# Levicoz/Options-model

Measured on AMD Instinct MI355X. Metric: paths x steps / sec (whole American pricing: path-gen + LSM + mean), higher is better.
Workload: dtype f32

## Files before the change

### include/omc.h

```cpp
#ifndef OMC_H
#define OMC_H

#include <stddef.h>
#include <stdint.h>

#ifdef __cplusplus
extern "C" {
#endif

#define OMC_ABI_VERSION 10

typedef struct omc_ctx omc_ctx;

enum {
    OMC_SEM_REFERENCE = 0,
    OMC_SEM_TEXTBOOK = 1,
    OMC_SEM_TWO_PASS = 2
};
enum { OMC_MODEL_GBM = 0, OMC_MODEL_HESTON = 1 };
enum {
    OMC_HESTON_REFERENCE_CLAMP = 0,
    OMC_HESTON_FULL_TRUNCATION = 1,
    OMC_HESTON_CALIBRATOR = 2
};

typedef struct {
    int32_t model;
    int32_t is_put;
    int32_t semantics;
    int32_t antithetic;
    int32_t heston_scheme;
    int32_t n_steps;
    int64_t n_paths;
    double S0, K, r, sigma, T;
    double v0, kappa, theta, xi, rho;
    uint64_t seed;
    uint64_t stream;
    uint64_t pair_offset;
} omc_params;

typedef struct {
    double price;
    double sum, sumsq;
    double std;
    double zero_prob;
    int64_t n_paths, n_exercised, n_zero, sum_nitm;
    double ms_paths, ms_lsm, ms_total;
    double ms_pass1, ms_pass2;
    int64_t timed;
    int64_t folded;
} omc_result;

int omc_abi_version(void);
const char* omc_last_error(void);
int omc_device_count(int* count);
int omc_ctx_device_info(omc_ctx* ctx, int* device, char* pci_bus_id, int pci_len, char* name, int name_len);
int omc_ctx_create(int device, void* hip_stream, omc_ctx** out);
int omc_ctx_destroy(omc_ctx* ctx);
int omc_sync(omc_ctx* ctx);
int omc_alloc(omc_ctx* ctx, size_t bytes, void** dptr);
int omc_free(omc_ctx* ctx, void* dptr);
int omc_memcpy_h2d(omc_ctx* ctx, void* dst, const void* src, size_t bytes);
int omc_memcpy_d2h(omc_ctx* ctx, void* dst, const void* src, size_t bytes);
int omc_set_option(omc_ctx* ctx, const char* key, int64_t value);
int omc_p2p_export(omc_ctx* ctx, void* handle_out, size_t bytes );
int omc_p2p_connect(omc_ctx* ctx, int rank, int world, const void* handles, size_t bytes );
int omc_p2p_disconnect(omc_ctx* ctx);
int omc_p2p_status(omc_ctx* ctx, int* connected, int* world, uint64_t* error_word);

int omc_gbm_paths_f32(omc_ctx* ctx, float* S, int64_t ld, int64_t n_paths, int n_steps, double S0,
                      double r, double sigma, double T, uint64_t seed, uint64_t stream,
                      uint64_t pair_offset, int antithetic);
int omc_heston_paths_f32(omc_ctx* ctx, float* S, int64_t ld, int64_t n_paths, int n_steps,
                         double S0, double r, double T, double v0, double kappa, double theta,
                         double xi, double rho, uint64_t seed, uint64_t stream,
                         uint64_t pair_offset, int scheme);
int omc_gbm_paths_from_normals_f32(omc_ctx* ctx, float* S, int64_t ld, int64_t n_paths,
                                   int n_steps, double S0, double r, double sigma, double T,
                                   const float* Zhalf, int64_t ldz, int antithetic);
int omc_heston_paths_from_normals_f32(omc_ctx* ctx, float* S, int64_t ld, int64_t n_paths,
                                      int n_steps, double S0, double r, double T, double v0,
                                      double kappa, double theta, double xi, double rho,
                                      const float* Z1half, const float* Z2half, int64_t ldz,
                                      int scheme);
int omc_philox4x32_10(omc_ctx* ctx, const uint32_t* in, uint32_t* out, int n);
int omc_gbm_normals_f32(omc_ctx* ctx, float* Z, int64_t ldz, int64_t n_pairs, int n_steps,
                        uint64_t seed, uint64_t stream, uint64_t pair_offset);

int omc_lsm_poly(omc_ctx* ctx, const float* S, int64_t ld, int64_t n_paths, int n_steps, double K,
                 double r, double T, int is_put, int semantics, omc_result* res,
                 double* betas_out, float* sx_out, int32_t* tex_out);
int omc_lsm_apply_frozen(omc_ctx* ctx, const float* S, int64_t ld, int64_t n_paths, int n_steps,
                         double K, double r, double T, int is_put, const double* betas,
                         omc_result* res, float* sx_out, int32_t* tex_out);

int omc_lsm_apply_values(omc_ctx* ctx, const float* S, int64_t ld, int64_t n_paths, int n_steps,
                         double K, double r, double T, int is_put, int semantics, const float* cont,
                         int64_t ldc, omc_result* res, float* sx_out, int32_t* tex_out);

int omc_lsm_contnet(omc_ctx* ctx, const float* S, int64_t ld, int64_t n_paths, int n_steps, double K, double r,
                    double T, int is_put, int nn_hidden, int nn_epochs, double nn_lr, uint64_t nn_seed,
                    omc_result* res, float* sx_out, int32_t* tex_out);
int omc_price_american_contnet(omc_ctx* ctx, const omc_params* p, int nn_hidden, int nn_epochs, double nn_lr,
                               uint64_t nn_seed, omc_result* res);
int omc_contnet_init_params(omc_ctx* ctx, int nn_hidden, int t, uint64_t nn_seed, float* params_out, int n);

typedef int (*omc_allreduce_fn)(void* user, double* dptr, int count);
int omc_set_allreduce_hook(omc_ctx* ctx, omc_allreduce_fn fn, void* user);

int omc_comm_unique_id(void* uid_out, size_t bytes);
int omc_comm_init(omc_ctx* ctx, int rank, int world, const void* uid, size_t bytes);
int omc_comm_destroy(omc_ctx* ctx);
int omc_comm_info(omc_ctx* ctx, int* rank, int* world);
int omc_comm_allreduce_f64(omc_ctx* ctx, double* host_inout, int count, int op);

int omc_price_american(omc_ctx* ctx, const omc_params* p, omc_result* res, float* S_keep,
                       int64_t ld);
typedef struct {
    omc_result base;
    double delta, gamma, vega, rho, theta;
    double se_delta, se_gamma, se_vega, se_rho, se_theta;
    double bump, price_up, price_down;
    int64_t n_exercised_up, n_exercised_down;
    double ms_greeks;
} omc_greeks;
int omc_price_american_greeks(omc_ctx* ctx, const omc_params* p, double bump, const double* betas, double* betas_out,
                              omc_greeks* out);
int omc_price_european(omc_ctx* ctx, const omc_params* p, omc_result* res);

int omc_heston_price_strikes(omc_ctx* ctx, int64_t n_paths, int n_steps, double S0, double r,
                             double T, double v0, double kappa, double theta, double xi, double rho,
                             uint64_t seed, uint64_t stream, int scheme, const double* strikes,
                             int n_strikes, int is_put, double* prices, double* stderrs);
int omc_heston_price_surface(omc_ctx* ctx, int64_t n_paths, int n_steps, double S0, double r, double v0, double kappa,
                             double theta, double xi, double rho, uint64_t seed, int scheme, const double* expiries,
                             const uint64_t* streams, int n_expiries, const double* strikes, const int32_t* expiry_of,
                             int n_quotes, int is_put, double* prices, double* stderrs);

int omc_mlp_param_count(int hidden, int layers);
int omc_lsm_apply_mlp(omc_ctx* ctx, const float* S, int64_t ld, int64_t n_paths, int n_steps, double K,
                      double r, double T, int is_put, int hidden, int layers, const float* params,
                      const double* feat_mean, const double* feat_std, double y_mean, double y_std,
                      double dropout, uint64_t seed, omc_result* res, float* sx_out, int32_t* tex_out);
int omc_lsm_apply_mlp_shard(omc_ctx* ctx, const float* S, int64_t ld, int64_t n_paths, int n_steps, double K,
                      double r, double T, int is_put, int hidden, int layers, const float* params,
                      const double* feat_mean, const double* feat_std, double y_mean, double y_std,
                      double dropout, uint64_t seed, omc_result* res, float* sx_out, int32_t* tex_out,
                            int64_t col_base0, int64_t col_base1);
int omc_nn_build_rows(omc_ctx* ctx, const float* S, int64_t ld, int64_t n_paths, int n_steps, double K,
                      double r, double T, int is_put, float* data, int64_t cap_rows, int64_t* n_rows,
                      double* stats16);
int omc_lsm_ols7(omc_ctx* ctx, const float* S, int64_t ld, int64_t n_paths, int n_steps, double K, double r, double T,
                 int is_put, omc_result* res, double* weights7, double* stats16, float* sx_out, int32_t* tex_out);
int omc_price_american_ols7(omc_ctx* ctx, const omc_params* p, omc_result* res, double* weights7, double* stats16);
int omc_nn_feature_stats(omc_ctx* ctx, const double* x, const int32_t* t, const double* y,
                         int64_t n_rows, double T, double dt, double* out16);
int omc_mlp_train_supported(int hidden, int layers, int64_t batch);
int omc_mlp_train_epoch(omc_ctx* ctx, const float* data, int64_t n_rows, int64_t batch, int hidden,
                        int layers, float* params, float* adam_m, float* adam_v, int64_t* step,
                        double lr, double beta1, double beta2, double eps, double weight_decay,
                        double dropout, uint64_t seed, uint64_t shuffle_key, double* mean_loss);
int omc_mlp_shuffle_indices(omc_ctx* ctx, int64_t n_rows, uint64_t shuffle_key, int64_t* out_device);
int omc_mlp_train_variant(int hidden, int layers, int64_t batch);
int omc_mlp_dropout_masks(omc_ctx* ctx, int variant, int hidden, int layers, int64_t n_rows, const uint32_t* keys,
                          uint32_t step, uint64_t seed, double dropout, uint8_t* out);

int omc_nn_half_counts(omc_ctx* ctx, const float* S, int64_t ld, int64_t n_paths, int n_steps, double K, int is_put,
                       int64_t* counts );
int omc_mlp_shard_epoch(omc_ctx* ctx, const float* data, int64_t n_rows_local, int64_t rows_global, int64_t batch,
                        uint64_t shuffle_key, const int64_t* gstart, const int64_t* lstart, int nseg,
                        int segs_per_step ,
                        float* data_epoch, uint32_t* drop_pos, int64_t* step_off);
int omc_mlp_train_epoch_sharded(omc_ctx* ctx, const float* data_epoch, int64_t n_rows_local, int64_t rows_global,
                                int64_t batch, int hidden, int layers, float* params, float* adam_m, float* adam_v,
                                int64_t* step, double lr, double beta1, double beta2, double eps, double weight_decay,
                                double dropout, uint64_t seed, const int64_t* step_off, const uint32_t* drop_pos,
                                double* mean_loss);

int omc_localvol_param_count(int hidden, int layers);
int omc_localvol_paths_f32(omc_ctx* ctx, float* S, int64_t ld, int64_t n_paths, int n_steps, double S0,
                           double r, double T, double K, int hidden, int layers, const float* params,
                           double m_scale, double tau_scale, double epsilon, const float* Z);

typedef struct {
    const float* data;
    int64_t n_rows, batch;
    float* params;
    float* adam_m;
    float* adam_v;
    int64_t step;
    double lr;
    uint64_t seed;
    uint64_t shuffle_key;
    double mean_loss;
} omc_mlp_job;
int omc_mlp_train_batch_supported(int hidden, int layers, int64_t batch);
int omc_mlp_train_epoch_batch(omc_ctx* ctx, omc_mlp_job* jobs, int n, int hidden, int layers, double beta1,
                              double beta2, double eps, double weight_decay, double dropout);

int omc_price_american_seq(omc_ctx* ctx, const omc_params* p, int n, omc_result* res);
int omc_seq_step_width(omc_ctx* ctx, const omc_params* p, int n);

int omc_price_american_batch(omc_ctx* ctx, const omc_params* p, int n, omc_result* res);
int omc_price_european_batch(omc_ctx* ctx, const omc_params* p, int n, omc_result* res);
int omc_price_american_contnet_batch(omc_ctx* ctx, const omc_params* p, int n, int nn_hidden, int nn_epochs,
                                     double nn_lr, const uint64_t* nn_seeds, omc_result* res);

#ifdef __cplusplus
}
#endif
#endif
```

### options_model_amd/_build.py

```python
from __future__ import annotations

import os
import shutil
import subprocess
import sys

_HERE = os.path.dirname(os.path.abspath(__file__))
CSRC = os.path.join(_HERE, "csrc")
LIBDIR = os.path.join(_HERE, "lib")
LIB = os.path.join(LIBDIR, "libomc.so")
SOURCES = ["omc_paths.hip", "omc_lsm.hip", "omc_batch.hip", "omc_mlp.hip", "omc_contnet.hip", "omc_rows.hip", "omc_ols7.hip", "omc_greeks.hip", "omc_comm.hip", "omc_p2p.hip",
           "omc_api.hip"]
HEADERS = ["omc_device.h", "omc_kernels.h", "omc_lsm_dev.h", "omc_paths_dev.h", "omc_contnet_dev.h", "omc_batch.h", "omc_greeks.h", "omc_comm.h", "omc_p2p.h",
           os.path.join("..", "..", "include", "omc.h")]
ARCH = "gfx950"
FLAGS_STAMP = os.path.join(LIBDIR, "libomc.flags")


def _flags() -> str:
    return " ".join(os.environ.get("OMC_HIPCC_FLAGS", "").split())


def _hipcc() -> str:
    for cand in (os.environ.get("HIPCC"), shutil.which("hipcc"), "/opt/rocm/bin/hipcc"):
        if cand and os.path.exists(cand):
            return cand
    raise RuntimeError("hipcc not found: libomc.so cannot be built (ROCm toolchain required)")


def _stale() -> bool:
    if not os.path.exists(LIB):
        return True
    try:
        built_with = open(FLAGS_STAMP).read().strip()
    except OSError:
        built_with = ""
    if built_with != _flags():
        return True
    t = os.path.getmtime(LIB)
    deps = [os.path.join(CSRC, s) for s in SOURCES + HEADERS] + [os.path.abspath(__file__)]
    return any(os.path.getmtime(d) > t for d in deps)


def build(force: bool = False, verbose: bool = False) -> str:
    if not force and not _stale():
        return LIB
    os.makedirs(LIBDIR, exist_ok=True)
    hipcc = _hipcc()
    objs = []
    procs = []
    for s in SOURCES:
        o = os.path.join(LIBDIR, s.replace(".hip", ".o"))
        cmd = [hipcc, f"--offload-arch={ARCH}", "-O3", "-std=c++17", "-fPIC", "-c",
               "-Wall", "-Wno-unused-function", os.path.join(CSRC, s), "-o", o]
        cmd[1:1] = _flags().split()
        if verbose:
            cmd.insert(1, "-Rpass-analysis=kernel-resource-usage")
            print(" ".join(cmd), flush=True)
        procs.append((cmd, subprocess.Popen(cmd)))
        objs.append(o)
    for cmd, p in procs:
        if p.wait() != 0:
            raise RuntimeError("hipcc failed: " + " ".join(cmd))
    for f in os.listdir(LIBDIR):
        if f.endswith(".o") and os.path.join(LIBDIR, f) not in objs:
            os.remove(os.path.join(LIBDIR, f))
    link = [hipcc, f"--offload-arch={ARCH}", "-shared", "-fPIC", "-o", LIB] + objs + ["-ldl"]
    if verbose:
        print(" ".join(link), flush=True)
    subprocess.check_call(link)
    with open(FLAGS_STAMP, "w") as f:
        f.write(_flags() + "\n")
    return LIB


if __name__ == "__main__":
    print(build(force="--force" in sys.argv, verbose="-v" in sys.argv))
```

### options_model_amd/_ffi.py

```python
from __future__ import annotations

import ctypes as C
import os
import threading

import numpy as np

from . import _build

ABI_VERSION = 10

SEMANTICS = {"reference": 0, "textbook": 1, "two_pass": 2}
MODELS = {"gbm": 0, "heston": 1}
HESTON_SCHEMES = {"reference": 0, "clamp": 0, "full_truncation": 1, "calibrator": 2}


class OmcError(RuntimeError):
    pass


class Params(C.Structure):
    _fields_ = [("model", C.c_int32), ("is_put", C.c_int32), ("semantics", C.c_int32),
                ("antithetic", C.c_int32), ("heston_scheme", C.c_int32), ("n_steps", C.c_int32),
                ("n_paths", C.c_int64),
                ("S0", C.c_double), ("K", C.c_double), ("r", C.c_double), ("sigma", C.c_double),
                ("T", C.c_double),
                ("v0", C.c_double), ("kappa", C.c_double), ("theta", C.c_double), ("xi", C.c_double),
                ("rho", C.c_double),
                ("seed", C.c_uint64), ("stream", C.c_uint64), ("pair_offset", C.c_uint64)]


class Result(C.Structure):
    _fields_ = [("price", C.c_double), ("sum", C.c_double), ("sumsq", C.c_double),
                ("std", C.c_double), ("zero_prob", C.c_double),
                ("n_paths", C.c_int64), ("n_exercised", C.c_int64), ("n_zero", C.c_int64),
                ("sum_nitm", C.c_int64),
                ("ms_paths", C.c_double), ("ms_lsm", C.c_double), ("ms_total", C.c_double),
                ("ms_pass1", C.c_double), ("ms_pass2", C.c_double), ("timed", C.c_int64),
                ("folded", C.c_int64)]

    def as_dict(self):
        return {k: getattr(self, k) for k, _ in self._fields_}


class Greeks(C.Structure):
    _fields_ = [("base", Result),
                ("delta", C.c_double), ("gamma", C.c_double), ("vega", C.c_double), ("rho", C.c_double),
                ("theta", C.c_double),
                ("se_delta", C.c_double), ("se_gamma", C.c_double), ("se_vega", C.c_double), ("se_rho", C.c_double),
                ("se_theta", C.c_double),
                ("bump", C.c_double), ("price_up", C.c_double), ("price_down", C.c_double),
                ("n_exercised_up", C.c_int64), ("n_exercised_down", C.c_int64),
                ("ms_greeks", C.c_double)]


class MlpJob(C.Structure):
    _fields_ = [("data", C.c_void_p), ("n_rows", C.c_int64), ("batch", C.c_int64),
                ("params", C.c_void_p), ("adam_m", C.c_void_p), ("adam_v", C.c_void_p),
                ("step", C.c_int64), ("lr", C.c_double), ("seed", C.c_uint64), ("shuffle_key", C.c_uint64),
                ("mean_loss", C.c_double)]


ALLREDUCE_FN = C.CFUNCTYPE(C.c_int, C.c_void_p, C.c_void_p, C.c_int)

_P, _I, _I64, _U64, _D, _SZ = C.c_void_p, C.c_int, C.c_int64, C.c_uint64, C.c_double, C.c_size_t
SIGNATURES = {
    "omc_abi_version": (C.c_int, []),
    "omc_last_error": (C.c_char_p, []),
    "omc_device_count": (C.c_int, [C.POINTER(C.c_int)]),
    "omc_ctx_create": (C.c_int, [_I, _P, C.POINTER(_P)]),
    "omc_ctx_destroy": (C.c_int, [_P]),
    "omc_sync": (C.c_int, [_P]),
    "omc_alloc": (C.c_int, [_P, _SZ, C.POINTER(_P)]),
    "omc_free": (C.c_int, [_P, _P]),
    "omc_memcpy_h2d": (C.c_int, [_P, _P, _P, _SZ]),
    "omc_memcpy_d2h": (C.c_int, [_P, _P, _P, _SZ]),
    "omc_set_option": (C.c_int, [_P, C.c_char_p, _I64]),
    "omc_gbm_paths_f32": (C.c_int, [_P, _P, _I64, _I64, _I, _D, _D, _D, _D, _U64, _U64, _U64, _I]),
    "omc_heston_paths_f32": (C.c_int, [_P, _P, _I64, _I64, _I] + [_D] * 8 + [_U64, _U64, _U64, _I]),
    "omc_gbm_paths_from_normals_f32": (C.c_int, [_P, _P, _I64, _I64, _I, _D, _D, _D, _D, _P, _I64, _I]),
    "omc_heston_paths_from_normals_f32": (C.c_int, [_P, _P, _I64, _I64, _I] + [_D] * 8 + [_P, _P, _I64, _I]),
    "omc_philox4x32_10": (C.c_int, [_P, _P, _P, _I]),
    "omc_gbm_normals_f32": (C.c_int, [_P, _P, _I64, _I64, _I, _U64, _U64, _U64]),
    "omc_lsm_poly": (C.c_int, [_P, _P, _I64, _I64, _I, _D, _D, _D, _I, _I, C.POINTER(Result), _P, _P, _P]),
    "omc_lsm_apply_frozen": (C.c_int, [_P, _P, _I64, _I64, _I, _D, _D, _D, _I, _P, C.POINTER(Result), _P, _P]),
    "omc_lsm_apply_values": (C.c_int, [_P, _P, _I64, _I64, _I, _D, _D, _D, _I, _I, _P, _I64, C.POINTER(Result), _P, _P]),
    "omc_lsm_contnet": (C.c_int, [_P, _P, _I64, _I64, _I, _D, _D, _D, _I, _I, _I, _D, _U64, C.POINTER(Result), _P, _P]),
    "omc_price_american_contnet": (C.c_int, [_P, C.POINTER(Params), _I, _I, _D, _U64, C.POINTER(Result)]),
    "omc_contnet_init_params": (C.c_int, [_P, _I, _I, _U64, _P, _I]),
    "omc_set_allreduce_hook": (C.c_int, [_P, ALLREDUCE_FN, _P]),
    "omc_comm_unique_id": (C.c_int, [_P, _SZ]),
    "omc_comm_init": (C.c_int, [_P, _I, _I, _P, _SZ]),
    "omc_comm_destroy": (C.c_int, [_P]),
    "omc_comm_info": (C.c_int, [_P, C.POINTER(C.c_int), C.POINTER(C.c_int)]),
    "omc_comm_allreduce_f64": (C.c_int, [_P, _P, _I, _I]),
    "omc_p2p_export": (C.c_int, [_P, _P, _SZ]),
    "omc_p2p_connect": (C.c_int, [_P, _I, _I, _P, _SZ]),
    "omc_p2p_disconnect": (C.c_int, [_P]),
    "omc_p2p_status": (C.c_int, [_P, C.POINTER(C.c_int), C.POINTER(C.c_int), C.POINTER(C.c_uint64)]),
    "omc_price_american": (C.c_int, [_P, C.POINTER(Params), C.POINTER(Result), _P, _I64]),
    "omc_price_american_greeks": (C.c_int, [_P, C.POINTER(Params), _D, _P, _P, C.POINTER(Greeks)]),
    "omc_price_european": (C.c_int, [_P, C.POINTER(Params), C.POINTER(Result)]),
    "omc_heston_price_strikes": (C.c_int, [_P, _I64, _I] + [_D] * 8 + [_U64, _U64, _I, _P, _I, _I, _P, _P]),
    "omc_heston_price_surface": (C.c_int, [_P, _I64, _I] + [_D] * 7 + [_U64, _I, _P, _P, _I, _P, _P, _I, _I, _P, _P]),
    "omc_price_american_seq": (C.c_int, [_P, C.POINTER(Params), _I, C.POINTER(Result)]),
    "omc_seq_step_width": (C.c_int, [_P, C.POINTER(Params), _I]),
    "omc_price_american_batch": (C.c_int, [_P, C.POINTER(Params), _I, C.POINTER(Result)]),
    "omc_price_european_batch": (C.c_int, [_P, C.POINTER(Params), _I, C.POINTER(Result)]),
    "omc_price_american_contnet_batch": (C.c_int, [_P, C.POINTER(Params), _I, _I, _I, _D, C.POINTER(C.c_uint64),
                                                   C.POINTER(Result)]),
    "omc_mlp_param_count": (C.c_int, [_I, _I]),
    "omc_mlp_train_supported": (C.c_int, [_I, _I, _I64]),
    "omc_mlp_train_epoch": (C.c_int, [_P, _P, _I64, _I64, _I, _I, _P, _P, _P, C.POINTER(C.c_int64)]
                            + [_D] * 6 + [_U64, _U64, C.POINTER(C.c_double)]),
    "omc_mlp_train_batch_supported": (C.c_int, [_I, _I, _I64]),
    "omc_mlp_train_epoch_batch": (C.c_int, [_P, C.POINTER(MlpJob), _I, _I, _I] + [_D] * 5),
    "omc_mlp_shuffle_indices": (C.c_int, [_P, _I64, _U64, _P]),
    "omc_mlp_train_variant": (C.c_int, [C.c_int, C.c_int, _I64]),
    "omc_price_american_ols7": (C.c_int, [_P, C.POINTER(Params), C.POINTER(Result), _P, _P]),
    "omc_lsm_ols7": (C.c_int, [_P, _P, _I64, _I64, _I, _D, _D, _D, _I, C.POINTER(Result), _P, _P, _P, _P]),
    "omc_ctx_device_info": (C.c_int, [_P, _P, _P, C.c_int, _P, C.c_int]),
    "omc_mlp_dropout_masks": (C.c_int, [_P, C.c_int, C.c_int, C.c_int, _I64, _P, C.c_uint32, _U64, C.c_double, _P]),
    "omc_nn_half_counts": (C.c_int, [_P, _P, _I64, _I64, _I, _D, _I, _P]),
    "omc_mlp_shard_epoch": (C.c_int, [_P, _P, _I64, _I64, _I64, _U64, _P, _P, _I, _I, _P, _P, _P]),
    "omc_mlp_train_epoch_sharded": (C.c_int, [_P, _P, _I64, _I64, _I64, _I, _I, _P, _P, _P, C.POINTER(C.c_int64)]
                                    + [_D] * 6 + [_U64, _P, _P, C.POINTER(C.c_double)]),
    "omc_lsm_apply_mlp": (C.c_int, [_P, _P, _I64, _I64, _I, _D, _D, _D, _I, _I, _I, _P, _P, _P, _D, _D, _D, _U64,
                                    C.POINTER(Result), _P, _P]),
    "omc_lsm_apply_mlp_shard": (C.c_int, [_P, _P, _I64, _I64, _I, _D, _D, _D, _I, _I, _I, _P, _P, _P, _D, _D, _D, _U64,
                                          C.POINTER(Result), _P, _P, _I64, _I64]),
    "omc_localvol_param_count": (C.c_int, [_I, _I]),
    "omc_localvol_paths_f32": (C.c_int, [_P, _P, _I64, _I64, _I, _D, _D, _D, _D, _I, _I, _P, _D, _D, _D, _P]),
    "omc_nn_build_rows": (C.c_int, [_P, _P, _I64, _I64, _I, _D, _D, _D, _I, _P, _I64, C.POINTER(C.c_int64), _P]),
    "omc_nn_feature_stats": (C.c_int, [_P, _P, _P, _P, _I64, _D, _D, _P]),
}

_lib = None
_lib_lock = threading.Lock()
_hip_runtime = None


def _preload_hip_runtime():
    global _hip_runtime
    if _hip_runtime is not None:
        return
    import importlib.util
    import sys
    mode = os.environ.get("OMC_HIP_RUNTIME", "auto")
    if mode == "system" or "torch" in sys.modules:
        return
    cand = None
    if mode not in ("auto", "torch") and os.path.exists(mode):
        cand = mode
    else:
        try:
            spec = importlib.util.find_spec("torch")
        except (ImportError, ValueError):
            spec = None
        if spec is not None and spec.submodule_search_locations:
            p = os.path.join(list(spec.submodule_search_locations)[0], "lib", "libamdhip64.so")
            if os.path.exists(p):
                cand = p
    if cand:
        try:
            _hip_runtime = C.CDLL(cand, mode=C.RTLD_GLOBAL)
        except OSError:
            _hip_runtime = None


def load_library(build_if_missing: bool = True):
    global _lib
    with _lib_lock:
        if _lib is not None:
            return _lib
        path = _build.LIB
        if not os.path.exists(path) or (build_if_missing and _build._stale()):
            if not build_if_missing:
                raise OmcError(f"{path} is missing: run `python -m options_model_amd._build`")
            try:
                path = _build.build()
            except Exception as e:
                if not os.path.exists(_build.LIB):
                    raise OmcError(f"libomc.so is missing and cannot be built: {e}") from e
                path = _build.LIB
        _preload_hip_runtime()
        lib = C.CDLL(path)
        for name, (res, args) in SIGNATURES.items():
            fn = getattr(lib, name)
            fn.restype = res
            fn.argtypes = args
        if lib.omc_abi_version() != ABI_VERSION:
            raise OmcError("libomc.so ABI version mismatch: rebuild the library")
        _lib = lib
        return lib


def _check(lib, rc):
    if rc == 0:
        return
    msg = (lib.omc_last_error() or b"").decode(errors="replace")
    if rc < 0:
        raise ValueError(msg)
    raise OmcError(f"HIP error {rc}: {msg}")


def comm_unique_id() -> bytes:
    lib = load_library()
    buf = C.create_string_buffer(128)
    _check(lib, lib.omc_comm_unique_id(buf, 128))
    return buf.raw


def device_count() -> int:
    lib = load_library()
    n = C.c_int(0)
    rc = lib.omc_device_count(C.byref(n))
    return n.value if rc == 0 else 0


class DeviceArray:

    def __init__(self, ctx, shape, dtype):
        self.ctx = ctx
        self.shape = tuple(int(s) for s in shape)
        self.dtype = np.dtype(dtype)
        self.nbytes = int(np.prod(self.shape)) * self.dtype.itemsize
        p = C.c_void_p()
        _check(ctx.lib, ctx.lib.omc_alloc(ctx.handle, self.nbytes, C.byref(p)))
        self.ptr = p.value
        ctx._arrays.add(self)

    def to_host(self):
        out = np.empty(self.shape, self.dtype)
        _check(self.ctx.lib, self.ctx.lib.omc_memcpy_d2h(self.ctx.handle, out.ctypes.data, self.ptr,
                                                          self.nbytes))
        return out

    def from_host(self, a):
        a = np.ascontiguousarray(a, self.dtype)
        assert a.shape == self.shape, (a.shape, self.shape)
        _check(self.ctx.lib, self.ctx.lib.omc_memcpy_h2d(self.ctx.handle, self.ptr, a.ctypes.data,
                                                          self.nbytes))
        return self

    def free(self):
        if self.ptr:
            self.ctx.lib.omc_free(self.ctx.handle, self.ptr)
            self.ptr = None
            self.ctx._arrays.discard(self)


class Context:

    def __init__(self, device: int = 0, stream: int | None = None):
# ... 97 lines not shown
        S = self.empty((N + 1, 2 * P), np.float32)
        _check(self.lib, self.lib.omc_heston_paths_from_normals_f32(
            self.handle, S.ptr, 2 * P, 2 * P, N, S0, r, T, v0, kappa, theta, xi, rho, z1.ptr, z2.ptr,
            P, scheme))
        z1.free()
        z2.free()
        return S

    def lsm_poly(self, S, K, r, T, is_put, semantics="reference", want_state=False, n_paths=None):
        N = S.shape[0] - 1
        ld = S.shape[1]
        M = ld if n_paths is None else n_paths
        res = Result()
        betas = np.zeros((N + 1, 4))
        sx = np.zeros(M, np.float32) if want_state else None
        tex = np.zeros(M, np.int32) if want_state else None
        ptr = S.ptr if isinstance(S, DeviceArray) else int(S.data_ptr())
        _check(self.lib, self.lib.omc_lsm_poly(self.handle, ptr, ld, M, N, K, r, T, int(is_put),
                                                SEMANTICS[semantics], C.byref(res), betas.ctypes.data,
                                                sx.ctypes.data if want_state else None,
                                                tex.ctypes.data if want_state else None))
        d = res.as_dict()
        d.update(betas=betas[:, :3], nitm=betas[:, 3].astype(np.int64), sx=sx, tex=tex)
        return d

    def lsm_ols7(self, S, K, r, T, is_put, want_state=False, n_paths=None):
        N = S.shape[0] - 1
        ld = S.shape[1]
        M = ld if n_paths is None else n_paths
        res = Result()
        w = np.zeros(7)
        st = np.zeros(16)
        sx = np.zeros(M, np.float32) if want_state else None
        tex = np.zeros(M, np.int32) if want_state else None
        ptr = S.ptr if isinstance(S, DeviceArray) else int(S.data_ptr())
        _check(self.lib, self.lib.omc_lsm_ols7(self.handle, ptr, ld, M, N, K, r, T, int(is_put), C.byref(res), w.ctypes.data,
                                                st.ctypes.data, sx.ctypes.data if want_state else None,
                                                tex.ctypes.data if want_state else None))
        d = res.as_dict()
        d.update(weights=w, feat_mean=st[:7].copy(), feat_std=st[7:14].copy(), y_mean=float(st[14]), y_std=float(st[15]),
                 sx=sx, tex=tex)
        return d

    def lsm_apply_frozen(self, S, K, r, T, is_put, betas4, want_state=True):
        N, M = S.shape[0] - 1, S.shape[1]
        b = np.ascontiguousarray(betas4, np.float64)
        assert b.shape == (N + 1, 4)
        res = Result()
        sx = np.zeros(M, np.float32) if want_state else None
        tex = np.zeros(M, np.int32) if want_state else None
        _check(self.lib, self.lib.omc_lsm_apply_frozen(self.handle, S.ptr, M, M, N, K, r, T,
                                                        int(is_put), b.ctypes.data, C.byref(res),
                                                        sx.ctypes.data if want_state else None,
                                                        tex.ctypes.data if want_state else None))
        d = res.as_dict()
        d.update(sx=sx, tex=tex)
        return d

    def lsm_apply_values(self, S, K, r, T, is_put, cont, semantics="reference", want_state=True):
        N, M = S.shape[0] - 1, S.shape[1]
        assert cont.shape == (N + 1, M) and cont.dtype == np.float32
        res = Result()
        sx = np.zeros(M, np.float32) if want_state else None
        tex = np.zeros(M, np.int32) if want_state else None
        _check(self.lib, self.lib.omc_lsm_apply_values(self.handle, S.ptr, M, M, N, K, r, T, int(is_put),
                                                        SEMANTICS[semantics], cont.ptr, M, C.byref(res),
                                                        sx.ctypes.data if want_state else None,
                                                        tex.ctypes.data if want_state else None))
        d = res.as_dict()
        d.update(sx=sx, tex=tex)
        return d

    def lsm_contnet(self, S, K, r, T, is_put, nn_hidden=32, nn_epochs=10, nn_lr=1e-3, nn_seed=0, want_state=True):
        N, M = S.shape[0] - 1, S.shape[1]
        res = Result()
        sx = np.zeros(M, np.float32) if want_state else None
        tex = np.zeros(M, np.int32) if want_state else None
        _check(self.lib, self.lib.omc_lsm_contnet(self.handle, S.ptr, M, M, N, K, r, T, int(is_put), int(nn_hidden),
                                                   int(nn_epochs), float(nn_lr), int(nn_seed) & (2**64 - 1),
                                                   C.byref(res), sx.ctypes.data if want_state else None,
                                                   tex.ctypes.data if want_state else None))
        d = res.as_dict()
        d.update(sx=sx, tex=tex)
        return d

    def contnet_init_params(self, nn_hidden, t, nn_seed=0):
        H = 32 if nn_hidden <= 32 else 64 if nn_hidden <= 64 else 128
        n = 8 * H + H * H + 2 * H + 1
        flat = np.zeros(n, np.float32)
        _check(self.lib, self.lib.omc_contnet_init_params(self.handle, int(nn_hidden), int(t),
                                                           int(nn_seed) & (2**64 - 1), flat.ctypes.data, n))
        h = int(nn_hidden)
        l0 = flat[:8 * H].reshape(H, 8)
        w1 = flat[8 * H:8 * H + H * H].reshape(H, H)
        b1 = flat[8 * H + H * H:8 * H + H * H + H]
        wo = flat[8 * H + H * H + H:8 * H + H * H + 2 * H]
        return dict(w0=l0[:h, :1].copy(), b0=l0[:h, 7].copy(), w1=w1[:h, :h].copy(), b1=b1[:h].copy(),
                    w2=wo[:h].reshape(1, h).copy(), b2=flat[-1:].copy(), flat=flat)

    def price_american_contnet(self, params: Params, nn_hidden=32, nn_epochs=10, nn_lr=1e-3, nn_seed=0):
        res = Result()
        _check(self.lib, self.lib.omc_price_american_contnet(self.handle, C.byref(params), int(nn_hidden),
                                                              int(nn_epochs), float(nn_lr),
                                                              int(nn_seed) & (2**64 - 1), C.byref(res)))
        return res.as_dict()

    def comm_init(self, rank: int, world: int, uid: bytes):
        buf = C.create_string_buffer(bytes(uid), 128)
        _check(self.lib, self.lib.omc_comm_init(self.handle, int(rank), int(world), buf, 128))

    def comm_destroy(self):
        _check(self.lib, self.lib.omc_comm_destroy(self.handle))

    def comm_info(self):
        r, w = C.c_int(0), C.c_int(0)
        _check(self.lib, self.lib.omc_comm_info(self.handle, C.byref(r), C.byref(w)))
        return r.value, w.value

    def device_info(self) -> dict:
        dev = C.c_int(-1)
        pci, name = C.create_string_buffer(64), C.create_string_buffer(256)
        _check(self.lib, self.lib.omc_ctx_device_info(self.handle, C.byref(dev), pci, 64, name, 256))
        return dict(device=dev.value, pci_bus_id=pci.value.decode(), name=name.value.decode())

    def comm_allreduce(self, values, op="sum"):
        a = np.ascontiguousarray(values, np.float64).copy()
        _check(self.lib, self.lib.omc_comm_allreduce_f64(self.handle, a.ctypes.data, a.size, 1 if op == "max" else 0))
        return a

    def p2p_export(self) -> bytes:
        buf = C.create_string_buffer(64)
        _check(self.lib, self.lib.omc_p2p_export(self.handle, buf, 64))
        return buf.raw

    def p2p_connect(self, rank: int, world: int, handles: bytes):
        buf = C.create_string_buffer(bytes(handles), 64 * int(world))
        _check(self.lib, self.lib.omc_p2p_connect(self.handle, int(rank), int(world), buf, 64 * int(world)))

    def p2p_disconnect(self):
        _check(self.lib, self.lib.omc_p2p_disconnect(self.handle))

    def p2p_status(self):
        a, b, e = C.c_int(0), C.c_int(0), C.c_uint64(0)
        _check(self.lib, self.lib.omc_p2p_status(self.handle, C.byref(a), C.byref(b), C.byref(e)))
        return bool(a.value), b.value, e.value

    def price_american(self, params: Params, keep_paths: DeviceArray | None = None):
        res = Result()
        _check(self.lib, self.lib.omc_price_american(
            self.handle, C.byref(params), C.byref(res), keep_paths.ptr if keep_paths else None,
            keep_paths.shape[1] if keep_paths else 0))
        return res.as_dict()

    def price_american_greeks(self, params: Params, bump=0.01, betas=None, want_betas=False):
        N = int(params.n_steps)
        b = None
        if betas is not None:
            b = np.ascontiguousarray(betas, np.float64)
            if b.shape != (N + 1, 4):
                raise ValueError(f"betas must have shape ({N + 1}, 4), got {b.shape}.")
        bo = np.zeros((N + 1, 4)) if want_betas else None
        g = Greeks()
        _check(self.lib, self.lib.omc_price_american_greeks(self.handle, C.byref(params), float(bump),
                                                             b.ctypes.data if b is not None else None,
                                                             bo.ctypes.data if bo is not None else None, C.byref(g)))
        d = g.base.as_dict()
        d.update({k: getattr(g, k) for k, _ in Greeks._fields_ if k != "base"})
        if want_betas:
            d["betas"] = bo
        return d

    def price_american_ols7(self, params: Params):
        res = Result()
        w, st = np.zeros(7), np.zeros(16)
        _check(self.lib, self.lib.omc_price_american_ols7(self.handle, C.byref(params), C.byref(res), w.ctypes.data,
                                                           st.ctypes.data))
        d = res.as_dict()
        d.update(weights=w, feat_mean=st[:7].copy(), feat_std=st[7:14].copy(), y_mean=float(st[14]), y_std=float(st[15]))
        return d

    def price_european(self, params: Params):
        res = Result()
        _check(self.lib, self.lib.omc_price_european(self.handle, C.byref(params), C.byref(res)))
        return res.as_dict()

    def heston_price_strikes(self, n_paths, n_steps, S0, r, T, v0, kappa, theta, xi, rho, strikes,
                             is_put=False, seed=42, stream=0, scheme=2):
        k = np.ascontiguousarray(strikes, np.float64)
        prices = np.empty_like(k)
        errs = np.empty_like(k)
        _check(self.lib, self.lib.omc_heston_price_strikes(
            self.handle, int(n_paths), int(n_steps), S0, r, T, v0, kappa, theta, xi, rho, int(seed),
            int(stream), int(scheme), k.ctypes.data, k.size, int(is_put), prices.ctypes.data,
            errs.ctypes.data))
        return prices, errs

    def heston_price_surface(self, n_paths, n_steps, S0, r, v0, kappa, theta, xi, rho, expiries, streams, strikes,
                             expiry_of, is_put=False, seed=42, scheme=2):
        T = np.ascontiguousarray(expiries, np.float64)
        st = np.ascontiguousarray(streams, np.uint64)
        k = np.ascontiguousarray(strikes, np.float64)
        eo = np.ascontiguousarray(expiry_of, np.int32)
        if st.shape != T.shape or eo.shape != k.shape or T.ndim != 1 or k.ndim != 1:
            raise ValueError("expiries / streams and strikes / expiry_of must be matching 1-d arrays")
        prices = np.empty_like(k)
        errs = np.empty_like(k)
        _check(self.lib, self.lib.omc_heston_price_surface(
            self.handle, int(n_paths), int(n_steps), S0, r, v0, kappa, theta, xi, rho, int(seed), int(scheme),
            T.ctypes.data, st.ctypes.data, T.size, k.ctypes.data, eo.ctypes.data, k.size, int(is_put), prices.ctypes.data,
            errs.ctypes.data))
        return prices, errs

    def mlp_train_epoch(self, data_ptr, n_rows, batch, params_ptr, m_ptr, v_ptr, step, lr, dropout, seed,
                        hidden=64, layers=2, beta1=0.9, beta2=0.999, eps=1e-8, weight_decay=1e-5,
                        shuffle_key=0):
        st = C.c_int64(int(step))
        loss = C.c_double(0.0)
        _check(self.lib, self.lib.omc_mlp_train_epoch(
            self.handle, int(data_ptr), int(n_rows), int(batch), int(hidden), int(layers), int(params_ptr),
            int(m_ptr), int(v_ptr), C.byref(st), float(lr), float(beta1), float(beta2), float(eps),
            float(weight_decay), float(dropout), int(seed), int(shuffle_key), C.byref(loss)))
        return loss.value, st.value

    def nn_half_counts(self, S_ptr, ld, n_paths, n_steps, K, is_put):
        out = np.zeros((max(int(n_steps) - 1, 0), 2), np.int64)
        _check(self.lib, self.lib.omc_nn_half_counts(self.handle, int(S_ptr), int(ld), int(n_paths), int(n_steps), float(K),
                                                     int(bool(is_put)), out.ctypes.data))
        return out

    def mlp_shard_epoch(self, data_ptr, n_rows_local, rows_global, batch, shuffle_key, gstart, lstart, data_epoch_ptr,
                        drop_pos_ptr, segs_per_step=0):
        g = np.ascontiguousarray(gstart, np.int64)
        l_ = np.ascontiguousarray(lstart, np.int64)
        assert g.size == l_.size + 1
        steps = (int(rows_global) + int(batch) - 1) // int(batch)
        so = np.zeros(steps + 1, np.int64)
        _check(self.lib, self.lib.omc_mlp_shard_epoch(
            self.handle, int(data_ptr) if n_rows_local else None, int(n_rows_local), int(rows_global), int(batch),
            int(shuffle_key), g.ctypes.data, l_.ctypes.data, int(l_.size), int(segs_per_step),
            int(data_epoch_ptr) if n_rows_local else None,
            int(drop_pos_ptr) if n_rows_local else None, so.ctypes.data))
        return so

    def mlp_train_epoch_sharded(self, data_epoch_ptr, n_rows_local, rows_global, batch, params_ptr, m_ptr, v_ptr, step, lr,
                                dropout, seed, step_off, drop_pos_ptr, hidden=64, layers=2, beta1=0.9, beta2=0.999,
                                eps=1e-8, weight_decay=1e-5):
        st = C.c_int64(int(step))
        loss = C.c_double(0.0)
        so = np.ascontiguousarray(step_off, np.int64)
        _check(self.lib, self.lib.omc_mlp_train_epoch_sharded(
            self.handle, int(data_epoch_ptr) if n_rows_local else None, int(n_rows_local), int(rows_global), int(batch),
            int(hidden), int(layers), int(params_ptr), int(m_ptr), int(v_ptr), C.byref(st), float(lr), float(beta1),
            float(beta2), float(eps), float(weight_decay), float(dropout), int(seed), so.ctypes.data,
            int(drop_pos_ptr) if n_rows_local else None, C.byref(loss)))
        return loss.value, st.value

    def mlp_train_epoch_batch(self, jobs, hidden, layers, dropout, beta1=0.9, beta2=0.999, eps=1e-8, weight_decay=1e-5):
        n = len(jobs)
        arr = (MlpJob * n)()
        for a, j in zip(arr, jobs):
            a.data, a.n_rows, a.batch = int(j["data_ptr"]), int(j["n_rows"]), int(j["batch"])
            a.params, a.adam_m, a.adam_v = int(j["params_ptr"]), int(j["m_ptr"]), int(j["v_ptr"])
            a.step, a.lr = int(j["step"]), float(j["lr"])
            a.seed, a.shuffle_key = int(j["seed"]) & (2**64 - 1), int(j["shuffle_key"]) & (2**64 - 1)
        _check(self.lib, self.lib.omc_mlp_train_epoch_batch(self.handle, arr, n, int(hidden), int(layers), float(beta1),
                                                            float(beta2), float(eps), float(weight_decay), float(dropout)))
        return [(a.mean_loss, a.step) for a in arr]

    def lsm_apply_mlp(self, S_ptr, ld, n_paths, n_steps, K, r, T, is_put, params_ptr, feat_mean, feat_std,
                      y_mean, y_std, dropout, seed, want_state=False, hidden=64, layers=2, col_bases=None):
        fm = np.ascontiguousarray(feat_mean, np.float64)
        fs = np.ascontiguousarray(feat_std, np.float64)
        assert fm.size == 7 and fs.size == 7
        res = Result()
        sx = np.empty(n_paths, np.float32) if want_state else None
        tex = np.empty(n_paths, np.int32) if want_state else None
        b0, b1 = (0, int(n_paths) // 2) if col_bases is None else (int(col_bases[0]), int(col_bases[1]))
        _check(self.lib, self.lib.omc_lsm_apply_mlp_shard(
            self.handle, int(S_ptr), int(ld), int(n_paths), int(n_steps), float(K), float(r), float(T),
            int(bool(is_put)), int(hidden), int(layers), int(params_ptr), fm.ctypes.data, fs.ctypes.data,
            float(y_mean), float(y_std), float(dropout), int(seed), C.byref(res),
            sx.ctypes.data if want_state else None, tex.ctypes.data if want_state else None, b0, b1))
        out = res.as_dict()
        if want_state:
            out["sx"], out["tex"] = sx, tex
        return out

    def nn_build_rows(self, S_ptr, ld, n_paths, n_steps, K, r, T, is_put, data_ptr=None, cap_rows=0):
        n = C.c_int64(0)
        st = np.zeros(16)
        _check(self.lib, self.lib.omc_nn_build_rows(
            self.handle, int(S_ptr), int(ld), int(n_paths), int(n_steps), float(K), float(r), float(T),
            int(bool(is_put)), int(data_ptr) if data_ptr else None, int(cap_rows), C.byref(n), st.ctypes.data))
        if not data_ptr:
            return n.value
        return n.value, st[:7].copy(), st[7:14].copy(), float(st[14]), float(st[15])

    def nn_feature_stats(self, x_ptr, t_ptr, y_ptr, n_rows, T, dt):
        out = np.zeros(16)
        _check(self.lib, self.lib.omc_nn_feature_stats(self.handle, int(x_ptr), int(t_ptr), int(y_ptr),
                                                       int(n_rows), float(T), float(dt), out.ctypes.data))
        return out[:7].copy(), out[8:15].copy()

    def mlp_dropout_masks(self, variant, hidden, layers, n_rows, step, seed, dropout, keys=None):
        out = np.zeros((int(layers), int(n_rows), int(hidden)), np.uint8)
        k = None if keys is None else np.ascontiguousarray(keys, np.uint32)
# ... 136 lines not shown
```

### options_model_amd/csrc/omc_api.hip

```cpp
#include <hip/hip_runtime.h>

#include <cmath>
#include <cstdio>
#include <cstring>
#include <functional>
#include <string>
#include <vector>

#include "../../include/omc.h"
#include <sched.h>

#include "omc_batch.h"
#include "omc_greeks.h"
#include "omc_comm.h"
#include "omc_p2p.h"
#include "omc_kernels.h"

namespace {

thread_local std::string g_err;

int fail(int code, const char* msg)
{
    g_err = msg;
    return code;
}

#define HIP_TRY(expr)                                                                      \
    do {                                                                                   \
        hipError_t e_ = (expr);                                                            \
        if (e_ != hipSuccess) {                                                            \
            char buf_[256];                                                                \
            snprintf(buf_, sizeof buf_, "%s failed: %s (%s:%d)", #expr, hipGetErrorString(e_), \
                     __FILE__, __LINE__);                                                  \
            g_err = buf_;                                                                  \
            return (int)e_ > 0 ? (int)e_ : 999;                                            \
        }                                                                                  \
    } while (0)

static size_t g_alloc_limit = 0;

struct DevBuf {
    void* p = nullptr;
    size_t cap = 0;
    int ensure(size_t bytes)
    {
        if (bytes <= cap) return 0;
        if (g_alloc_limit && bytes > g_alloc_limit) {
            g_err = "hipMalloc refused: " + std::to_string(bytes) + " bytes asked for, option alloc_limit is " +
                    std::to_string(g_alloc_limit) + " (out of memory)";
            return (int)hipErrorOutOfMemory;
        }
        if (p) {
            hipError_t e = hipFree(p);
            p = nullptr;
            cap = 0;
            if (e != hipSuccess) return (int)e;
        }
        size_t want = bytes + bytes / 8 + 256;
        hipError_t e = hipMalloc(&p, want);
        if (e != hipSuccess) {
            (void)hipGetLastError();
            want = bytes;
            e = hipMalloc(&p, want);
        }
        if (e != hipSuccess) {
            (void)hipGetLastError();
            g_err = std::string("hipMalloc failed: ") + hipGetErrorString(e);
            p = nullptr;
            return (int)e;
        }
        cap = want;
        return 0;
    }
    void release()
    {
        if (p) (void)hipFree(p);
        p = nullptr;
        cap = 0;
    }
};

}

struct RowsCache {
    bool valid = false;
    const float* S = nullptr;
    int64_t ld = 0, M = 0;
    int N = 0, is_put = 0;
    double K = 0, r = 0, T = 0;
    int64_t R = 0;
    double st[16] = {0};
};

constexpr size_t kVoteBytes = 1024;

struct omc_ctx {
    int device = 0;
    hipStream_t stream = nullptr;
    bool own_stream = false;
    DevBuf S, sx, tex, ex, D, part, gmom, betas, part1, result, scratch, sweep_args;
    DevBuf bslab, btable, bres, bdisc;
    DevBuf mlp_part, mlp_loss, mlp_wt;
    DevBuf mlp_gred, shard;
    DevBuf cn_scratch, cn_data, cn_net, cn_cont;
    std::vector<char> h_table;
    std::vector<double> h_disc, h_bres;
    std::vector<double> hD;
    int D_N = -1;
    double D_r = 0, D_T = 0;
    const double* D_ptr = nullptr;
    double hres[8];
    double* hres_pin = nullptr;
    double* hres_dev = nullptr;
    double *seq_pin = nullptr, *seq_dev = nullptr;
    int seq_cap = 0;
    hipEvent_t ev_seq = nullptr;
    hipEvent_t ev_entry = nullptr;
    hipEvent_t ev[7] = {nullptr, nullptr, nullptr, nullptr, nullptr, nullptr, nullptr};
    std::vector<hipEvent_t> ev_pool;
    int seq_event_stride = 0;
    DevBuf mS, mstate, mtable;
    DevBuf mb_slab, mb_table, mb_bc;
    std::vector<double> mb_bc_host;
    double mb_beta1 = -1.0, mb_beta2 = -1.0;
    size_t mb_bc_cap = 0;
    char* mtab_pin = nullptr;
    int mtab_slot = 0;
    int seq_step_k = -1;
    int seq_step_wgs = 0;
    int gbm_vec = 0, heston_vec = 0;
    int fold = 1;
    DevBuf foldC;
    DevBuf gk_part, gk_res;
    struct FoldKey { int N = -1; double c0 = 0, g = 0; } fold_key[2];
    int world = 1;
    omc_allreduce_fn hook = nullptr;
    void* hook_user = nullptr;
    omc::Comm* comm = nullptr;
    omc::P2P* p2p = nullptr;
    int p2p_use = 1;
    bool p2p_used = false;
    double p2p_deadline_s = 2.0;
    double p2p_first_deadline_s = 30.0;
    hipStream_t comm_stream = nullptr;
    hipEvent_t ev_moments[2] = {nullptr, nullptr}, ev_reduced[2] = {nullptr, nullptr};
    RowsCache rows_cache;
    DevBuf S2, seq_local, part1b, gmomb, seq_vote;
    int seq_overlap = -1;
    bool defer_result_allreduce = false;
    hipGraph_t sweep_graph = nullptr;
    hipGraphExec_t sweep_exec = nullptr;
    int64_t sg_M = -1, sg_ld = -1;
    int sg_N = -1, sg_sem = -1, sg_vec4 = -1, sg_failed = 0;
    const void* sg_args = nullptr;
    std::vector<char> sweep_img;
    char* sweep_pin = nullptr;
    int sweep_pin_slot = 0;
    int step_graph = -1;
    int device_cus = 0;
    bool distributed() const { return comm != nullptr || hook != nullptr; }
};

namespace {

int check_market(double S0, double K, double T, double r)
{
    if (!(S0 > 0) || !(K > 0) || !(T > 0)) return fail(-1, "S0, K, T must be positive.");
    if (!(r >= 0)) return fail(-2, "r must be non-negative.");
    return 0;
}

int check_sizes(int64_t n_paths, int n_steps)
{
    if (n_paths <= 0 || n_steps <= 0)
        return fail(-3, "num_simulations and num_time_steps must be positive integers.");
    if (n_steps > omc::kMaxSteps) return fail(-8, "num_time_steps exceeds the supported maximum (4094).");
    return 0;
}

int check_matrix(const void* S, int64_t ld, int64_t n_paths)
{
    if (!S) return fail(-7, "null path matrix pointer.");
    if (ld < n_paths) return fail(-6, "leading dimension smaller than n_paths.");
    return 0;
}

int bind(omc_ctx* c)
{
    if (!c) return fail(-7, "null context.");
    c->rows_cache.valid = false;
    HIP_TRY(hipSetDevice(c->device));
    return 0;
}

int bind_in(omc_ctx* c)
{
    int rc = bind(c);
    if (rc) return rc;
    if (!c->own_stream) return 0;
    if (!c->ev_entry) HIP_TRY(hipEventCreateWithFlags(&c->ev_entry, hipEventDisableTiming));
    HIP_TRY(hipEventRecord(c->ev_entry, nullptr));
    HIP_TRY(hipStreamWaitEvent(c->stream, c->ev_entry, 0));
    return 0;
}

int wait_stream(omc_ctx* c)
{
    timespec t0, t1;
    clock_gettime(CLOCK_MONOTONIC, &t0);
    for (int i = 0;; ++i) {
        const hipError_t q = hipStreamQuery(c->stream);
        if (q == hipSuccess) return 0;
        if (q != hipErrorNotReady) HIP_TRY(q);
        if ((i & 15) == 15) {
            clock_gettime(CLOCK_MONOTONIC, &t1);
            const double us = (t1.tv_sec - t0.tv_sec) * 1e6 + (t1.tv_nsec - t0.tv_nsec) * 1e-3;
            if (us > 2000.0) break;
            if (us > 50.0) sched_yield();
        }
    }
    HIP_TRY(hipStreamSynchronize(c->stream));
    return 0;
}

int prepare_lsm(omc_ctx* c, int64_t M, int N, double r, double T, bool two_pass,
                bool clear_tables, omc::LsmWorkspace* w)
{
    int rc;
    if ((rc = c->sx.ensure(sizeof(float) * (size_t)M))) return rc;
    if ((rc = c->tex.ensure(sizeof(int32_t) * (size_t)M))) return rc;
    if ((rc = c->ex.ensure(sizeof(float) * (size_t)M + 16))) return rc;
    if ((rc = c->D.ensure(sizeof(double) * (size_t)(N + 1)))) return rc;
    if ((rc = c->part.ensure(sizeof(double) * 2 * 8 * omc::kMaxLsmBlocks))) return rc;
    if ((rc = c->gmom.ensure(sizeof(double) * 8 * (size_t)(N + 1)))) return rc;
    if ((rc = c->betas.ensure(sizeof(double) * 4 * (size_t)(N + 1)))) return rc;
    if ((rc = c->result.ensure(sizeof(double) * 8))) return rc;
    w->part1 = nullptr;
    w->part1_tiles = 0;
    if (two_pass) {
        const size_t tiles = omc::lsm_part1_tiles(M);
        if ((rc = c->part1.ensure(sizeof(double) * 8 * (size_t)(N + 1) * tiles))) return rc;
        w->part1 = (double*)c->part1.p;
        w->part1_tiles = (int64_t)tiles;
    }
    w->sx = (float*)c->sx.p;
    w->tex = (int32_t*)c->tex.p;
    w->live = (float*)c->ex.p;
    w->D = (double*)c->D.p;
    w->part = (double*)c->part.p;
    w->gmom = (double*)c->gmom.p;
    w->betas = (double*)c->betas.p;
    w->result = (double*)c->result.p;
    if (c->D_N != N || c->D_r != r || c->D_T != T || c->D_ptr != w->D) {
        c->hD.resize((size_t)N + 1);
        const double dt = T / N;
        for (int k = 0; k <= N; ++k) c->hD[(size_t)k] = std::exp(-r * dt * (double)k);
        HIP_TRY(hipMemcpyAsync(w->D, c->hD.data(), sizeof(double) * (size_t)(N + 1),
                               hipMemcpyHostToDevice, c->stream));
        HIP_TRY(hipStreamSynchronize(c->stream));
        c->D_N = N; c->D_r = r; c->D_T = T; c->D_ptr = w->D;
    }
    if (clear_tables) {
        HIP_TRY(hipMemsetAsync(w->gmom, 0, sizeof(double) * 8 * (size_t)(N + 1), c->stream));
        HIP_TRY(hipMemsetAsync(w->betas, 0, sizeof(double) * 4 * (size_t)(N + 1), c->stream));
    }
    return 0;
}

int allreduce(omc_ctx* c, double* dptr, int count)
{
    if (c->comm) {
        std::string err;
        const int rc = omc::comm_allreduce_f64(c->comm, dptr, (size_t)count, 0, c->stream, &err);
        if (rc) return fail(rc, err.c_str());
        return 0;
    }
    if (c->hook) {
        if (c->hook(c->hook_user, dptr, count)) return fail(998, "all-reduce hook failed");
    }
    return 0;
}

int allreduce_host(omc_ctx* c, double* dev, double* host, int n)
{
    int rc;
    HIP_TRY(hipMemcpyAsync(dev, host, sizeof(double) * (size_t)n, hipMemcpyHostToDevice, c->stream));
    if ((rc = allreduce(c, dev, n))) return rc;
    HIP_TRY(hipMemcpyAsync(host, dev, sizeof(double) * (size_t)n, hipMemcpyDeviceToHost, c->stream));
    HIP_TRY(hipStreamSynchronize(c->stream));
    return 0;
}

bool p2p_active(const omc_ctx* c)
{
    return c->p2p && c->p2p_use && omc::p2p_connected(c->p2p) && c->distributed() && omc::p2p_world(c->p2p) == c->world;
}

bool step_graph_enabled(const omc_ctx* c)
{
    if (c->step_graph >= 0) return c->step_graph != 0;
    static const int env = [] {
        const char* e = getenv("OMC_STEP_GRAPH");
        return e ? atoi(e) : 0;
    }();
    return env != 0;
}

void drop_sweep_graph(omc_ctx* c)
{
    if (c->sweep_exec) (void)hipGraphExecDestroy(c->sweep_exec);
    if (c->sweep_graph) (void)hipGraphDestroy(c->sweep_graph);
    c->sweep_exec = nullptr;
    c->sweep_graph = nullptr;
    c->sg_M = -1;
}

constexpr int kNoGraph = -12345;
int enqueue_sweep_graph(omc_ctx* c, const omc::LsmProblem& p, const omc::LsmWorkspace& w, int semantics,
                        bool fill_state)
{
    if (c->sg_failed) return kNoGraph;
    const size_t nb = omc::lsm_sweep_args_bytes();
    constexpr int kSlots = 32;
    if (c->sweep_args.ensure(nb)) return kNoGraph;
    if (!c->sweep_pin && hipHostMalloc((void**)&c->sweep_pin, nb * kSlots, hipHostMallocDefault) != hipSuccess) {
        c->sweep_pin = nullptr;
        c->sg_failed = 1;
        (void)hipGetLastError();
        return kNoGraph;
    }
    std::vector<char> img(nb);
    omc::lsm_sweep_args_image(p, w, semantics, fill_state, img.data());
    if (img != c->sweep_img) {
        if (c->sweep_pin_slot == kSlots) {
            HIP_TRY(hipStreamSynchronize(c->stream));
            c->sweep_pin_slot = 0;
        }
        char* slot = c->sweep_pin + nb * (size_t)c->sweep_pin_slot++;
        memcpy(slot, img.data(), nb);
        HIP_TRY(hipMemcpyAsync(c->sweep_args.p, slot, nb, hipMemcpyHostToDevice, c->stream));
        c->sweep_img.swap(img);
    }
    const int vec4 = ((p.M % 4) == 0 && (p.ld % 4) == 0 && ((uintptr_t)p.S % 16) == 0) ? 1 : 0;
    if (!c->sweep_exec || c->sg_M != p.M || c->sg_N != p.N || c->sg_sem != semantics || c->sg_vec4 != vec4 ||
        c->sg_ld != p.ld || c->sg_args != c->sweep_args.p) {
        drop_sweep_graph(c);
        bool ok = hipStreamBeginCapture(c->stream, hipStreamCaptureModeThreadLocal) == hipSuccess;
        if (ok) {
            const hipError_t le = omc::lsm_sweep_indirect(c->stream, p, w, semantics, c->sweep_args.p);
            const hipError_t ee = hipStreamEndCapture(c->stream, &c->sweep_graph);
            ok = le == hipSuccess && ee == hipSuccess && c->sweep_graph != nullptr;
        }
        if (ok) ok = hipGraphInstantiate(&c->sweep_exec, c->sweep_graph, nullptr, nullptr, 0) == hipSuccess;
        if (!ok) {
            (void)hipGetLastError();
            drop_sweep_graph(c);
            c->sg_failed = 1;
            return kNoGraph;
        }
        c->sg_M = p.M; c->sg_N = p.N; c->sg_sem = semantics; c->sg_vec4 = vec4; c->sg_ld = p.ld;
        c->sg_args = c->sweep_args.p;
    }
    HIP_TRY(hipGraphLaunch(c->sweep_exec, c->stream));
    return 0;
}

int enqueue_lsm(omc_ctx* c, const omc::LsmProblem& p, const omc::LsmWorkspace& w, int semantics,
                bool write_state)
{
    hipStream_t st = c->stream;
    int rc;
    if (semantics == OMC_SEM_TWO_PASS) {
        HIP_TRY(omc::lsm_pass1_moments(st, p, w));
        if (c->distributed() && (rc = allreduce(c, w.gmom, 8 * (p.N + 1)))) return rc;
        HIP_TRY(omc::lsm_pass2_apply(st, p, w, write_state, true));
    } else {
        const bool ext = c->distributed();
        const bool flags = semantics == OMC_SEM_REFERENCE;
        int graphed = kNoGraph;
        if (!ext && step_graph_enabled(c)) {
            graphed = enqueue_sweep_graph(c, p, w, semantics, write_state);
            if (graphed != 0 && graphed != kNoGraph) return graphed;
        }
        if (graphed == kNoGraph) {
            const int nblk = omc::lsm_sweep_blocks(p.M);
            if (ext && p2p_active(c)) omc::p2p_begin_call(c->p2p);
            for (int t = p.N; t >= 1; --t) {
                HIP_TRY(omc::lsm_step(st, p, w, semantics, t, ext));
                if (ext && t >= 2) {
                    if (p2p_active(c)) {
                        HIP_TRY(omc::p2p_exchange_step(c->p2p, st, w, t - 1, nblk));
                        c->p2p_used = true;
                    } else {
                        HIP_TRY(omc::lsm_reduce_step_moments(st, w, t - 1, nblk));
                        if ((rc = allreduce(c, w.gmom + (size_t)(t - 1) * 8, 8))) return rc;
                    }
                }
            }
            HIP_TRY(omc::lsm_final_reduce(st, p, w, semantics == OMC_SEM_TEXTBOOK ? 0 : 1, flags, write_state));
        }
    }
    if (c->p2p_used) HIP_TRY(omc::p2p_stamp_results(c->p2p, st, w.result, 1));
    if (c->distributed() && !c->defer_result_allreduce && (rc = allreduce(c, w.result, 8))) return rc;
    return 0;
}

int check_p2p(omc_ctx* c, const double* h = nullptr, int n = 0)
{
    if (!c->p2p_used) return 0;
    c->p2p_used = false;
    unsigned long long w = 0;
    HIP_TRY(omc::p2p_error_word(c->p2p, c->stream, &w));
    bool peer = false;
    for (int i = 0; h && i < n; ++i) peer = peer || h[(size_t)i * 8 + 6] != 0.0;
    if (w == 1)
        return fail(3100, "direct peer exchange of the per-step moments timed out (a peer's contribution never arrived); "
                          "omc_p2p_disconnect and use the collective");
    if (w || peer)
        return fail(3100, "direct peer exchange of the per-step moments: another rank gave up on an exchange (its deadline "
                          "ran out), so this job's sums are not to be trusted; omc_p2p_disconnect and use the collective");
    return 0;
}

void fill_result(omc_result* res, const double* h, int64_t M, int world = 1)
{
    res->sum = h[0];
    res->sumsq = h[1];
    res->n_paths = M;
    res->n_exercised = (int64_t)llround(h[2]);
    res->n_zero = (int64_t)llround(h[3]);
    res->sum_nitm = (int64_t)llround(h[4] / (double)world);
    res->price = h[0] / (double)M;
    const double var = h[1] / (double)M - res->price * res->price;
    res->std = var > 0 ? std::sqrt(var) : 0.0;
    res->zero_prob = (double)res->n_zero / (double)M;
}

int copy_outputs(omc_ctx* c, const omc::LsmWorkspace& w, int64_t M, int N, double* betas_out,
                 float* sx_out, int32_t* tex_out)
{
    if (betas_out)
        HIP_TRY(hipMemcpyAsync(betas_out, w.betas, sizeof(double) * 4 * (size_t)(N + 1),
                               hipMemcpyDeviceToHost, c->stream));
    if (sx_out)
        HIP_TRY(hipMemcpyAsync(sx_out, w.sx, sizeof(float) * (size_t)M, hipMemcpyDeviceToHost, c->stream));
    if (tex_out)
        HIP_TRY(hipMemcpyAsync(tex_out, w.tex, sizeof(int32_t) * (size_t)M, hipMemcpyDeviceToHost,
                               c->stream));
    return 0;
}

}

extern "C" {

int omc_abi_version(void) { return OMC_ABI_VERSION; }

const char* omc_last_error(void) { return g_err.c_str(); }

int omc_device_count(int* count)
{
    if (!count) return fail(-7, "null pointer.");
    int n = 0;
    hipError_t e = hipGetDeviceCount(&n);
    if (e != hipSuccess) {
        *count = 0;
        (void)hipGetLastError();
        g_err = std::string("hipGetDeviceCount: ") + hipGetErrorString(e);
        return (int)e;
    }
    *count = n;
    return 0;
}

int omc_ctx_create(int device, void* hip_stream, omc_ctx** out)
{
    if (!out) return fail(-7, "null pointer.");
    *out = nullptr;
    int n = 0;
    HIP_TRY(hipGetDeviceCount(&n));
    if (device < 0 || device >= n) return fail(-4, "no such HIP device.");
    HIP_TRY(hipSetDevice(device));
    omc_ctx* c = new omc_ctx();
    c->device = device;
    auto undo = [&](hipError_t e) {
        for (auto& ev : c->ev)
            if (ev) (void)hipEventDestroy(ev);
        if (c->own_stream && c->stream) (void)hipStreamDestroy(c->stream);
        delete c;
        return e;
    };
    if (hip_stream) {
        c->stream = (hipStream_t)hip_stream;
        c->own_stream = false;
    } else {
        const hipError_t e = hipStreamCreateWithFlags(&c->stream, hipStreamNonBlocking);
        if (e != hipSuccess) {
            c->stream = nullptr;
            HIP_TRY(undo(e));
        }
        c->own_stream = true;
    }
    for (auto& ev : c->ev) {
        const hipError_t e = hipEventCreate(&ev);
        if (e != hipSuccess) {
            ev = nullptr;
            HIP_TRY(undo(e));
        }
    }
    if (hipHostMalloc((void**)&c->hres_pin, sizeof(double) * 8, hipHostMallocMapped) != hipSuccess ||
        hipHostGetDevicePointer((void**)&c->hres_dev, c->hres_pin, 0) != hipSuccess) {
        (void)hipGetLastError();
        if (c->hres_pin) (void)hipHostFree(c->hres_pin);
        c->hres_pin = c->hres_dev = nullptr;
    }
    (void)hipDeviceGetAttribute(&c->device_cus, hipDeviceAttributeMultiprocessorCount, device);
    *out = c;
    return 0;
}

int omc_ctx_destroy(omc_ctx* c)
{
    if (!c) return 0;
    (void)hipSetDevice(c->device);
    (void)hipStreamSynchronize(c->stream);
    drop_sweep_graph(c);
    if (c->comm) omc::comm_destroy(c->comm);
    c->comm = nullptr;
    if (c->p2p) omc::p2p_destroy(c->p2p);
    c->p2p = nullptr;
    for (DevBuf* b : {&c->S, &c->sx, &c->tex, &c->ex, &c->D, &c->part, &c->gmom, &c->betas, &c->part1,
                      &c->result, &c->scratch, &c->sweep_args, &c->bslab, &c->btable, &c->bres, &c->bdisc,
                      &c->mlp_part, &c->mlp_loss, &c->mlp_wt, &c->mlp_gred, &c->shard, &c->S2, &c->seq_local, &c->part1b, &c->gmomb, &c->seq_vote, &c->cn_scratch, &c->cn_data, &c->cn_net, &c->cn_cont,
                      &c->mS, &c->mstate, &c->mtable, &c->mb_slab, &c->mb_table, &c->mb_bc})
        b->release();
    if (c->sweep_pin) (void)hipHostFree(c->sweep_pin);
    if (c->mtab_pin) (void)hipHostFree(c->mtab_pin);
    if (c->comm_stream) (void)hipStreamDestroy(c->comm_stream);
    for (int b = 0; b < 2; ++b) {
        if (c->ev_moments[b]) (void)hipEventDestroy(c->ev_moments[b]);
        if (c->ev_reduced[b]) (void)hipEventDestroy(c->ev_reduced[b]);
    }
    for (auto& ev : c->ev)
        if (ev) (void)hipEventDestroy(ev);
    for (auto& ev : c->ev_pool)
        if (ev) (void)hipEventDestroy(ev);
    if (c->hres_pin) (void)hipHostFree(c->hres_pin);
    if (c->seq_pin) (void)hipHostFree(c->seq_pin);
    if (c->ev_seq) (void)hipEventDestroy(c->ev_seq);
    if (c->ev_entry) (void)hipEventDestroy(c->ev_entry);
    if (c->own_stream && c->stream) (void)hipStreamDestroy(c->stream);
    delete c;
    return 0;
}

int omc_ctx_device_info(omc_ctx* c, int* device, char* pci_bus_id, int pci_len, char* name, int name_len)
{
    int rc = bind(c);
    if (rc) return rc;
    if (device) *device = c->device;
    if (pci_bus_id && pci_len > 0) {
        pci_bus_id[0] = 0;
        HIP_TRY(hipDeviceGetPCIBusId(pci_bus_id, pci_len, c->device));
    }
    if (name && name_len > 0) {
        hipDeviceProp_t prop;
        HIP_TRY(hipGetDeviceProperties(&prop, c->device));
        snprintf(name, (size_t)name_len, "%s", prop.name);
    }
    return 0;
}

int omc_sync(omc_ctx* c)
{
    int rc = bind(c);
    if (rc) return rc;
    HIP_TRY(hipStreamSynchronize(c->stream));
    return 0;
}

int omc_alloc(omc_ctx* c, size_t bytes, void** dptr)
{
    int rc = bind(c);
    if (rc) return rc;
    if (!dptr) return fail(-7, "null pointer.");
    HIP_TRY(hipMalloc(dptr, bytes ? bytes : 1));
    return 0;
}

int omc_free(omc_ctx* c, void* dptr)
{
    int rc = bind_in(c);
    if (rc) return rc;
    if (dptr) {
        HIP_TRY(hipStreamSynchronize(c->stream));
        HIP_TRY(hipFree(dptr));
    }
    return 0;
}

int omc_memcpy_h2d(omc_ctx* c, void* dst, const void* src, size_t bytes)
{
    int rc = bind_in(c);
    if (rc) return rc;
    if (!bytes) return 0;
    HIP_TRY(hipMemcpyAsync(dst, src, bytes, hipMemcpyHostToDevice, c->stream));
    HIP_TRY(hipStreamSynchronize(c->stream));
    return 0;
}

int omc_memcpy_d2h(omc_ctx* c, void* dst, const void* src, size_t bytes)
{
    int rc = bind_in(c);
    if (rc) return rc;
    if (!bytes) return 0;
    HIP_TRY(hipMemcpyAsync(dst, src, bytes, hipMemcpyDeviceToHost, c->stream));
    HIP_TRY(hipStreamSynchronize(c->stream));
    return 0;
}

int omc_set_option(omc_ctx* c, const char* key, int64_t value)
{
    if (!c || !key) return fail(-7, "null pointer.");
    if (!strcmp(key, "gbm_vec")) c->gbm_vec = (int)value;
    else if (!strcmp(key, "alloc_limit")) g_alloc_limit = value > 0 ? (size_t)value : 0;
    else if (!strcmp(key, "fold_antithetic")) c->fold = value <= 0 ? 0 : (value >= 2 ? 2 : 1);
    else if (!strcmp(key, "heston_vec")) c->heston_vec = (int)value;
    else if (!strcmp(key, "world_size")) c->world = value > 0 ? (int)value : 1;
    else if (!strcmp(key, "step_graph")) c->step_graph = value < 0 ? -1 : (value ? 1 : 0);
    else if (!strcmp(key, "seq_overlap")) c->seq_overlap = value < 0 ? -1 : (value ? 1 : 0);
    else if (!strcmp(key, "seq_event_stride")) c->seq_event_stride = value > 0 ? (int)value : 0;
    else if (!strcmp(key, "seq_step_k")) c->seq_step_k = value < 0 ? -1 : (int)(value > 32 ? 32 : value);
    else if (!strcmp(key, "seq_step_wgs")) c->seq_step_wgs = value > 0 ? (int)value : 0;
    else if (!strcmp(key, "p2p_exchange")) c->p2p_use = value ? 1 : 0;
    else if (!strcmp(key, "p2p_deadline_ms") || !strcmp(key, "p2p_first_deadline_ms")) {
        if (value <= 0) return fail(-4, "a p2p deadline must be positive.");
        (key[4] == 'f' ? c->p2p_first_deadline_s : c->p2p_deadline_s) = (double)value * 1e-3;
        if (c->p2p) omc::p2p_set_deadline(c->p2p, c->p2p_deadline_s, c->p2p_first_deadline_s);
    }
    else return fail(-4, "unknown option key.");
    return 0;
}

int omc_set_allreduce_hook(omc_ctx* c, omc_allreduce_fn fn, void* user)
{
    if (!c) return fail(-7, "null context.");
    if (fn) {
        int rc;
        if ((rc = bind(c))) return rc;
        if ((rc = c->seq_vote.ensure(kVoteBytes))) return rc;
    }
    c->hook = fn;
    c->hook_user = user;
    return 0;
}

int omc_comm_unique_id(void* uid_out, size_t bytes)
{
    if (!uid_out || bytes < (size_t)omc::kCommUidBytes) return fail(-7, "unique-id buffer must hold 128 bytes.");
    std::string err;
    const int rc = omc::comm_unique_id(uid_out, &err);
    if (rc) return fail(rc, err.c_str());
    return 0;
}

int omc_comm_init(omc_ctx* c, int rank, int world, const void* uid, size_t bytes)
{
    int rc;
    if ((rc = bind(c))) return rc;
    if (!uid || bytes < (size_t)omc::kCommUidBytes) return fail(-7, "unique id must be 128 bytes.");
    if (world < 1 || rank < 0 || rank >= world) return fail(-4, "rank / world size out of range.");
    if (c->comm) return fail(-4, "this context already has a communicator.");
    std::string err;
    omc::Comm* comm = nullptr;
    if ((rc = c->seq_vote.ensure(kVoteBytes))) return rc;
    rc = omc::comm_create(rank, world, uid, &comm, &err);
    if (rc) return fail(rc, err.c_str());
    c->comm = comm;
    c->world = omc::comm_world(comm);
    return 0;
}

int omc_comm_destroy(omc_ctx* c)
{
    int rc;
    if ((rc = bind(c))) return rc;
    if (!c->comm) return 0;
    HIP_TRY(hipStreamSynchronize(c->stream));
    omc::comm_destroy(c->comm);
    c->comm = nullptr;
    c->world = 1;
    return 0;
}

int omc_comm_info(omc_ctx* c, int* rank, int* world)
{
    if (!c) return fail(-7, "null context.");
    if (rank) *rank = omc::comm_rank(c->comm);
    if (world) *world = c->comm ? omc::comm_world(c->comm) : 0;
    return 0;
}

int omc_comm_allreduce_f64(omc_ctx* c, double* host_inout, int count, int op)
{
    int rc;
    if ((rc = bind(c))) return rc;
    if (!c->comm) return fail(-4, "no communicator on this context (omc_comm_init).");
    if (!host_inout || count <= 0 || count > 4096) return fail(-7, "bad buffer (1..4096 doubles).");
    if (op != 0 && op != 1) return fail(-4, "op must be 0 (sum) or 1 (max).");
    if ((rc = c->scratch.ensure(sizeof(double) * 4096))) return rc;
    double* d = (double*)c->scratch.p;
    HIP_TRY(hipMemcpyAsync(d, host_inout, sizeof(double) * (size_t)count, hipMemcpyHostToDevice, c->stream));
    std::string err;
    rc = omc::comm_allreduce_f64(c->comm, d, (size_t)count, op, c->stream, &err);
    if (rc) return fail(rc, err.c_str());
    HIP_TRY(hipMemcpyAsync(host_inout, d, sizeof(double) * (size_t)count, hipMemcpyDeviceToHost, c->stream));
    HIP_TRY(hipStreamSynchronize(c->stream));
    return 0;
}

int omc_p2p_export(omc_ctx* c, void* handle_out, size_t bytes)
{
    int rc;
    if ((rc = bind(c))) return rc;
    if (!handle_out || bytes < (size_t)omc::kP2PHandleBytes) return fail(-7, "handle buffer must hold 64 bytes.");
    if (c->p2p) return fail(-4, "this context already has a mailbox (omc_p2p_disconnect first).");
    std::string err;
    omc::P2P* p = nullptr;
    rc = omc::p2p_export(&p, handle_out, &err);
    if (rc) return fail(rc, err.c_str());
    c->p2p = p;
    omc::p2p_set_deadline(p, c->p2p_deadline_s, c->p2p_first_deadline_s);
    return 0;
}

int omc_p2p_connect(omc_ctx* c, int rank, int world, const void* handles, size_t bytes)
{
    int rc;
    if ((rc = bind(c))) return rc;
    if (!c->p2p) return fail(-4, "no mailbox on this context (omc_p2p_export first).");
    if (!handles || world < 1 || bytes < (size_t)world * omc::kP2PHandleBytes)
        return fail(-7, "handles must hold world x 64 bytes, in rank order.");
    std::string err;
    rc = omc::p2p_connect(c->p2p, rank, world, handles, &err);
    if (rc) return fail(rc, err.c_str());
    return 0;
}

int omc_p2p_disconnect(omc_ctx* c)
{
    int rc;
    if ((rc = bind(c))) return rc;
    if (!c->p2p) return 0;
    HIP_TRY(hipStreamSynchronize(c->stream));
    omc::p2p_destroy(c->p2p);
    c->p2p = nullptr;
    c->p2p_used = false;
    return 0;
}

int omc_p2p_status(omc_ctx* c, int* connected, int* world, uint64_t* error_word)
{
    int rc;
    if ((rc = bind(c))) return rc;
    if (connected) *connected = (c->p2p && omc::p2p_connected(c->p2p)) ? 1 : 0;
    if (world) *world = c->p2p ? omc::p2p_world(c->p2p) : 0;
    if (error_word) {
        *error_word = 0;
        if (c->p2p && omc::p2p_connected(c->p2p)) {
            unsigned long long w = 0;
            HIP_TRY(omc::p2p_error_word(c->p2p, c->stream, &w));
            *error_word = w;
        }
    }
    return 0;
}

int omc_gbm_paths_f32(omc_ctx* c, float* S, int64_t ld, int64_t n_paths, int n_steps, double S0,
                      double r, double sigma, double T, uint64_t seed, uint64_t stream,
// ... 187 lines not shown
    int rc;
    if (!p) return fail(-7, "null params.");
    if ((rc = check_market(p->S0, p->K, p->T, p->r))) return rc;
    if ((rc = check_sizes(p->n_paths, p->n_steps))) return rc;
    if (p->model == OMC_MODEL_GBM) {
        if (!(p->sigma > 0)) return fail(-5, "S0, K, T, and sigma must be positive.");
    } else if (p->model == OMC_MODEL_HESTON) {
        if (!(p->rho >= -1.0 && p->rho <= 1.0) || !(p->v0 >= 0)) return fail(-5, "invalid Heston parameters.");
        if (p->heston_scheme < 0 || p->heston_scheme > 2) return fail(-4, "unknown Heston scheme.");
        if (!p->antithetic) return fail(-4, "Heston paths are always antithetic.");
    } else {
        return fail(-4, "unknown model.");
    }
    if (p->semantics < 0 || p->semantics > 2) return fail(-4, "unknown semantics.");
    if (p->antithetic && (p->n_paths & 1)) return fail(-3, "antithetic layout needs an even n_paths.");
    return 0;
}

static int enqueue_paths(omc_ctx* c, const omc_params* p, float* S, int64_t ld, bool fold = false)
{
    if (p->model == OMC_MODEL_GBM)
        HIP_TRY(omc::launch_gbm_paths(c->stream, S, ld, fold ? p->n_paths / 2 : p->n_paths, p->n_steps, p->S0, p->r,
                                      p->sigma, p->T, p->seed, (uint32_t)p->stream, p->pair_offset,
                                      fold ? 0 : p->antithetic, c->gbm_vec));
    else
        HIP_TRY(omc::launch_heston_paths(c->stream, S, ld, p->n_paths, p->n_steps, p->S0, p->r, p->T, p->v0,
                                         p->kappa, p->theta, p->xi, p->rho, p->seed, (uint32_t)p->stream,
                                         p->pair_offset, p->heston_scheme, c->heston_vec));
    return 0;
}

constexpr int64_t kFoldMinPaths = 65536;
static bool fold_applies(const omc_ctx* c, const omc_params* p)
{
    if (!c->fold || p->model != OMC_MODEL_GBM || !p->antithetic || p->semantics != OMC_SEM_TWO_PASS) return false;
    return c->fold >= 2 || p->n_paths * (int64_t)(c->world > 0 ? c->world : 1) >= kFoldMinPaths;
}

static int plan_storage(omc_ctx* c, const omc_params* p, int slot, int64_t* ld, const double** cK)
{
    *cK = nullptr;
    *ld = (p->n_paths + 63) / 64 * 64;
    if (!fold_applies(c, p)) return 0;
    int rc;
    const size_t per = (size_t)omc::kMaxSteps + 2;
    if ((rc = c->foldC.ensure(sizeof(double) * 2 * per))) return rc;
    double* tab = (double*)c->foldC.p + per * (size_t)slot;
    double c0, g;
    omc::gbm_fold_constants(p->S0, p->K, p->r, p->sigma, p->T, p->n_steps, &c0, &g);
    omc_ctx::FoldKey& key = c->fold_key[slot];
    if (key.N != p->n_steps || key.c0 != c0 || key.g != g) {
        HIP_TRY(omc::lsm_fold_table(c->stream, tab, p->n_steps, c0, g));
        key.N = p->n_steps; key.c0 = c0; key.g = g;
    }
    *ld = (p->n_paths / 2 + 63) / 64 * 64;
    *cK = tab;
    return 0;
}

static int enqueue_pricing(omc_ctx* c, const omc_params* p, float* S_keep, int64_t ld, double* result_dev,
                           hipEvent_t* evs, double** result_out)
{
    const bool timed = evs != nullptr;
    int rc;
    const int64_t M = p->n_paths;
    const int N = p->n_steps;
    float* S = S_keep;
    const double* cK = nullptr;
    if (S) {
        if (ld < M) return fail(-6, "leading dimension smaller than n_paths.");
    } else {
        if ((rc = plan_storage(c, p, 0, &ld, &cK))) return rc;
        if ((rc = c->S.ensure(sizeof(float) * (size_t)ld * (size_t)(N + 1)))) return rc;
        S = (float*)c->S.p;
    }
    omc::LsmWorkspace w;
    if ((rc = prepare_lsm(c, M, N, p->r, p->T, p->semantics == OMC_SEM_TWO_PASS, false, &w))) return rc;
    omc::LsmProblem prob{S, ld, M, N, p->is_put ? 1 : 0, p->K, p->r, p->T};
    prob.fold_cK = cK;
    if (timed) {
        w.ev_p1_end = evs[4]; w.ev_p2_begin = evs[5]; w.ev_p2_end = evs[6];
        HIP_TRY(hipEventRecord(evs[0], c->stream));
    }
    if ((rc = enqueue_paths(c, p, S, ld, cK != nullptr))) return rc;
    if (timed) HIP_TRY(hipEventRecord(evs[1], c->stream));
    if (result_dev) w.result = result_dev;
    if ((rc = enqueue_lsm(c, prob, w, p->semantics, false))) return rc;
    if (result_out) *result_out = w.result;
    return 0;
}

static int read_kernel_times(const hipEvent_t* evs, const omc_params* p, omc_result* res, bool has_end = true)
{
    float ms = 0;
    HIP_TRY(hipEventElapsedTime(&ms, evs[0], evs[1]));
    res->ms_paths = ms;
    if (has_end) {
        HIP_TRY(hipEventElapsedTime(&ms, evs[1], evs[2]));
        res->ms_lsm = ms;
        res->ms_total = res->ms_paths + res->ms_lsm;
    }
    if (p->semantics == OMC_SEM_TWO_PASS && p->n_steps >= 2) {
        HIP_TRY(hipEventElapsedTime(&ms, evs[1], evs[4]));
        res->ms_pass1 = ms;
        HIP_TRY(hipEventElapsedTime(&ms, evs[5], evs[6]));
        res->ms_pass2 = ms;
    }
    return 0;
}

static int sample_events(omc_ctx* c, int s, hipEvent_t** out)
{
    if (s == 0) {
        *out = c->ev;
        return 0;
    }
    const size_t need = 7 * (size_t)s;
    while (c->ev_pool.size() < need) {
        hipEvent_t e = nullptr;
        HIP_TRY(hipEventCreate(&e));
        c->ev_pool.push_back(e);
    }
    *out = c->ev_pool.data() + 7 * (size_t)(s - 1);
    return 0;
}

static inline int seq_sample_index(const omc_ctx* c, int i)
{
    if (i == 0) return 0;
    const int k = c->seq_event_stride;
    return (k > 0 && i % k == 0) ? i / k : -1;
}

int omc_price_american(omc_ctx* c, const omc_params* p, omc_result* res, float* S_keep, int64_t ld)
{
    int rc;
    if ((rc = S_keep ? bind_in(c) : bind(c))) return rc;
    if ((rc = check_params(p))) return rc;
    if (!res) return fail(-7, "null result pointer.");
    const bool zero_copy = c->hres_dev && !c->distributed();
    double* hres = c->hres_pin ? c->hres_pin : c->hres;
    double* result = nullptr;
    if ((rc = enqueue_pricing(c, p, S_keep, ld, zero_copy ? c->hres_dev : nullptr, c->ev, &result))) return rc;
    HIP_TRY(hipEventRecord(c->ev[2], c->stream));
    if (!zero_copy)
        HIP_TRY(hipMemcpyAsync(hres, result, sizeof(double) * 8, hipMemcpyDeviceToHost, c->stream));
    if ((rc = wait_stream(c))) return rc;
    if ((rc = check_p2p(c, hres, 1))) return rc;
    memset(res, 0, sizeof *res);
    fill_result(res, hres, c->distributed() ? p->n_paths * c->world : p->n_paths,
                c->distributed() ? c->world : 1);
    res->folded = (!S_keep && fold_applies(c, p)) ? 1 : 0;
    return read_kernel_times(c->ev, p, res);
}

int omc_price_american_greeks(omc_ctx* c, const omc_params* p, double bump, const double* betas, double* betas_out,
                              omc_greeks* out)
{
    int rc;
    if ((rc = bind(c))) return rc;
    if (!out) return fail(-7, "null result pointer.");
    if ((rc = check_params(p))) return rc;
    if (p->semantics != OMC_SEM_TWO_PASS) return fail(-4, "Greeks are those of the two-pass flow (semantics 2).");
    if (!(bump > 0.0 && bump <= 0.5)) return fail(-4, "bump must lie in (0, 0.5].");
    if (c->distributed()) return fail(-10, "the Greeks sweep runs on one GPU.");
    const int64_t M = p->n_paths;
    const int N = p->n_steps;
    int64_t ld = 0;
    const double* cK = nullptr;
    if ((rc = plan_storage(c, p, 0, &ld, &cK))) return rc;
    if ((rc = c->S.ensure(sizeof(float) * (size_t)ld * (size_t)(N + 1)))) return rc;
    float* S = (float*)c->S.p;
    omc::LsmWorkspace w;
    if ((rc = prepare_lsm(c, M, N, p->r, p->T, betas == nullptr, betas_out != nullptr, &w))) return rc;
    if (betas) {
        HIP_TRY(hipMemcpyAsync(w.betas, betas, sizeof(double) * 4 * (size_t)(N + 1), hipMemcpyHostToDevice, c->stream));
        HIP_TRY(hipStreamSynchronize(c->stream));
    }
    omc::GreeksArgs g;
    g.S = S; g.ld = ld; g.cols = cK ? M / 2 : M;
    g.N = N; g.is_put = p->is_put ? 1 : 0; g.gbm = p->model == OMC_MODEL_GBM ? 1 : 0;
    g.K = p->K; g.S0 = p->S0; g.r = p->r; g.sigma = p->sigma; g.T = p->T; g.h = bump;
    g.D = w.D; g.betas = w.betas; g.cK = cK; g.gmom = betas ? nullptr : w.gmom;
    const int64_t nblk = omc::greeks_blocks(g);
    if ((rc = c->gk_part.ensure(sizeof(double) * omc::kGreeksQ * (size_t)nblk))) return rc;
    if ((rc = c->gk_res.ensure(sizeof(double) * omc::kGreeksQ))) return rc;
    g.part = (double*)c->gk_part.p;
    g.result = (double*)c->gk_res.p;
    omc::LsmProblem prob{S, ld, M, N, p->is_put ? 1 : 0, p->K, p->r, p->T};
    prob.fold_cK = cK;
    w.ev_p1_end = c->ev[4];
    HIP_TRY(hipEventRecord(c->ev[0], c->stream));
    if ((rc = enqueue_paths(c, p, S, ld, cK != nullptr))) return rc;
    HIP_TRY(hipEventRecord(c->ev[1], c->stream));
    const bool fit = betas == nullptr && N >= 2;
    if (fit) {
        HIP_TRY(omc::lsm_pass1_moments(c->stream, prob, w));
        HIP_TRY(omc::lsm_solve_betas(c->stream, w.gmom, w.betas, N));
    }
    HIP_TRY(omc::lsm_greeks(c->stream, g, c->ev[5], c->ev[6]));
    HIP_TRY(hipEventRecord(c->ev[2], c->stream));
    double h[omc::kGreeksQ];
    HIP_TRY(hipMemcpyAsync(h, g.result, sizeof h, hipMemcpyDeviceToHost, c->stream));
    if (betas_out) {
        if (betas) memcpy(betas_out, betas, sizeof(double) * 4 * (size_t)(N + 1));
        else HIP_TRY(hipMemcpyAsync(betas_out, w.betas, sizeof(double) * 4 * (size_t)(N + 1), hipMemcpyDeviceToHost, c->stream));
    }
    if ((rc = wait_stream(c))) return rc;
    memset(out, 0, sizeof *out);
    fill_result(&out->base, h, M);
    out->base.folded = cK ? 1 : 0;
    const double Md = (double)M;
    auto mean_se = [&](int q, double* mean, double* se) {
        *mean = h[q] / Md;
        const double var = h[q + 1] / Md - *mean * *mean;
        *se = std::sqrt((var > 0.0 ? var : 0.0) / Md);
    };
    mean_se(8, &out->delta, &out->se_delta);
    mean_se(10, &out->gamma, &out->se_gamma);
    if (g.gbm) {
        mean_se(12, &out->vega, &out->se_vega);
        mean_se(14, &out->rho, &out->se_rho);
        mean_se(16, &out->theta, &out->se_theta);
    } else {
        out->vega = out->rho = out->theta = NAN;
        out->se_vega = out->se_rho = out->se_theta = NAN;
    }
    out->bump = bump;
    out->price_up = h[5] / Md;
    out->price_down = h[6] / Md;
    out->n_exercised_up = (int64_t)llround(h[18]);
    out->n_exercised_down = (int64_t)llround(h[19]);
    float ms = 0;
    HIP_TRY(hipEventElapsedTime(&ms, c->ev[0], c->ev[1]));
    out->base.ms_paths = ms;
    HIP_TRY(hipEventElapsedTime(&ms, c->ev[1], c->ev[2]));
    out->base.ms_lsm = ms;
    out->base.ms_total = out->base.ms_paths + out->base.ms_lsm;
    if (fit) {
        HIP_TRY(hipEventElapsedTime(&ms, c->ev[1], c->ev[4]));
        out->base.ms_pass1 = ms;
    }
    HIP_TRY(hipEventElapsedTime(&ms, c->ev[5], c->ev[6]));
    out->ms_greeks = ms;
    return 0;
}

namespace {

int contnet_sweep(omc_ctx* c, const omc::LsmProblem& p, omc::LsmWorkspace& w, int hidden, int epochs, double lr,
                  uint64_t seed, double* rows_total)
{
    int rc;
    const int H = omc::cn_padded_width(hidden);
    const int np = omc::mlp_train_param_count(H, 2);
    const int64_t M = p.M;
    const int N = p.N;
    if ((rc = c->cn_scratch.ensure(omc::cn_scratch_bytes(M)))) return rc;
    if ((rc = c->cn_net.ensure(sizeof(float) * 3 * (size_t)np))) return rc;
    if ((rc = c->cn_cont.ensure(sizeof(float) * (size_t)M))) return rc;
    if ((rc = c->mlp_wt.ensure(omc::mlp_wt_bytes(H, 2)))) return rc;
    if ((rc = c->mlp_loss.ensure(sizeof(double)))) return rc;
    HIP_TRY(hipMemsetAsync(c->mlp_loss.p, 0, sizeof(double), c->stream));
    float* net = (float*)c->cn_net.p;
    w.cont = (const float*)c->cn_cont.p;
    w.ldc = 0;
    const double* hdr_dev = omc::cn_header(p, c->cn_scratch.p);
    *rows_total = 0.0;
    HIP_TRY(omc::lsm_step(c->stream, p, w, OMC_SEM_REFERENCE, N, false));
    for (int t = N - 1; t >= 1; --t) {
        const double Dt = c->hD[(size_t)(N - t)];
        HIP_TRY(omc::cn_count(c->stream, p, w, c->cn_scratch.p, t, Dt));
        double hdr[4];
        HIP_TRY(hipMemcpyAsync(hdr, hdr_dev, sizeof hdr, hipMemcpyDeviceToHost, c->stream));
        HIP_TRY(hipStreamSynchronize(c->stream));
        const int64_t R = (int64_t)hdr[0];
        if (R <= 0) continue;
        *rows_total += (double)R;
        if ((rc = c->cn_data.ensure(sizeof(float) * 8 * (size_t)R))) return rc;
        if ((rc = c->mlp_part.ensure(omc::mlp_partial_bytes(H, 2, R)))) return rc;
        HIP_TRY(omc::cn_rows(c->stream, p, w, c->cn_scratch.p, t, Dt, (float*)c->cn_data.p));
        HIP_TRY(omc::cn_init(c->stream, hidden, t, seed, net, net + np, net + 2 * (size_t)np));
        omc::MlpTrainPlan plan;
        plan.data = (const float*)c->cn_data.p;
        plan.params = net; plan.adam_m = net + np; plan.adam_v = net + 2 * (size_t)np;
        plan.partial = (float*)c->mlp_part.p; plan.loss_acc = (double*)c->mlp_loss.p;
        plan.nrows = R; plan.batch = R; plan.hidden = H; plan.layers = 2;
        plan.wt = (float*)c->mlp_wt.p;
        plan.lr = lr; plan.beta1 = 0.9; plan.beta2 = 0.999; plan.eps = 1e-8;
        plan.weight_decay = 0.0; plan.dropout = 0.0; plan.seed = 0; plan.shuffle_key = 0;
        for (int e = 0; e < epochs; ++e) {
            plan.first_step = e;
            plan.wt_current = e > 0;
            HIP_TRY(omc::mlp_train_steps(c->stream, plan));
        }
        HIP_TRY(omc::cn_forward(c->stream, p, w, c->cn_scratch.p, t, Dt, hidden, net, (float*)c->cn_cont.p));
        HIP_TRY(omc::lsm_step(c->stream, p, w, OMC_SEM_REFERENCE, t, false));
    }
    return 0;
}

int check_contnet(omc_ctx* c, int hidden, int epochs, double lr)
{
    if (hidden < 1 || omc::cn_padded_width(hidden) < 0) return fail(-4, "nn_hidden must be in 1 .. 128.");
    if (epochs < 0) return fail(-4, "nn_epochs must be non-negative.");
    if (!(lr > 0.0)) return fail(-4, "nn_lr must be positive.");
// ... 1463 lines not shown
```

### options_model_amd/csrc/omc_kernels.h

```cpp
#pragma once
#include <hip/hip_runtime.h>
#include <stdint.h>

#include <atomic>
#include <cmath>

namespace omc {

inline hipError_t set_max_dynamic_lds(std::atomic<uint64_t>& mask, const void* kernel, size_t bytes)
{
    int dev = 0;
    hipError_t e = hipGetDevice(&dev);
    if (e != hipSuccess) return e;
    const uint64_t bit = 1ull << (dev & 63);
    if (mask.load(std::memory_order_acquire) & bit) return hipSuccess;
    e = hipFuncSetAttribute(kernel, hipFuncAttributeMaxDynamicSharedMemorySize, (int)bytes);
    if (e != hipSuccess) return e;
    mask.fetch_or(bit, std::memory_order_release);
    return hipSuccess;
}

hipError_t launch_gbm_paths(hipStream_t st, float* S, int64_t ld, int64_t n_paths, int n_steps,
                            double S0, double r, double sigma, double T, uint64_t seed,
                            uint32_t stream, uint64_t pair_offset, int antithetic, int vec_hint);
hipError_t launch_heston_paths(hipStream_t st, float* S, int64_t ld, int64_t n_paths, int n_steps,
                               double S0, double r, double T, double v0, double kappa,
                               double theta, double xi, double rho, uint64_t seed, uint32_t stream,
                               uint64_t pair_offset, int scheme, int vec_hint);
hipError_t launch_gbm_from_normals(hipStream_t st, float* S, int64_t ld, int64_t n_paths,
                                   int n_steps, double S0, double r, double sigma, double T,
                                   const float* Z, int64_t ldz, int antithetic);
hipError_t launch_heston_from_normals(hipStream_t st, float* S, int64_t ld, int64_t n_paths,
                                      int n_steps, double S0, double r, double T, double v0,
                                      double kappa, double theta, double xi, double rho,
                                      const float* Z1, const float* Z2, int64_t ldz, int scheme);
hipError_t launch_heston_terminal_store(hipStream_t st, float* ST, int64_t n_paths, int n_steps,
                                        double S0, double r, double T, double v0, double kappa,
                                        double theta, double xi, double rho, uint64_t seed,
                                        uint32_t stream, uint64_t pair_offset, int scheme);
size_t payoff_partial_bytes(int64_t n_paths, int n_quotes);
hipError_t launch_payoff_means(hipStream_t st, const float* ST, int64_t n_paths, const double* K_dev,
                               int n_strikes, int is_put, double* part_dev, double* out_dev);
size_t heston_surface_table_bytes(int n_expiries);
void heston_surface_fill_table(void* tab_host, int n_steps, double r, const double* T_host, const uint32_t* stream_host,
                               int n_expiries, double kappa, double theta, double xi, double rho);
hipError_t launch_heston_terminal_surface(hipStream_t st, float* ST, int64_t ldst, int64_t n_paths, int n_steps, double S0,
                                          int n_expiries, double v0, uint64_t seed, uint64_t pair_offset, int scheme,
                                          const void* tab_dev);
hipError_t launch_payoff_means_surface(hipStream_t st, const float* ST, int64_t ldst, int64_t n_paths, const double* K_dev,
                                       const int32_t* expiry_of_dev, int n_quotes, int is_put, double* part_dev, double* out_dev);
hipError_t launch_philox_kat(hipStream_t st, const uint32_t* in, uint32_t* out, int n);
hipError_t launch_gbm_normals(hipStream_t st, float* Z, int64_t ldz, int64_t n_pairs, int n_steps,
                              uint64_t seed, uint32_t stream, uint64_t pair_offset);

constexpr int kMaxLsmBlocks = 1024;
hipError_t launch_terminal(hipStream_t st, double* part, int* nblk_out, int model, int scheme,
                           int antithetic, int64_t n_paths, int n_steps, double S0, double K,
                           double r, double sigma, double T, double v0, double kappa, double theta,
                           double xi, double rho, int is_put, uint64_t seed, uint32_t stream,
                           uint64_t pair_offset);

constexpr int kMaxSteps = 4094;

struct LsmProblem {
    const float* S;
    int64_t ld, M;
    int N, is_put;
    double K, r, T;
    const double* fold_cK = nullptr;
};

struct LsmWorkspace {
    float* sx;
    int32_t* tex;
    float* live;
    double* D;
    double* part;
    double* gmom;
    int gstride = 8;
    double* betas;
    double* part1;
    int64_t part1_tiles;
    double* result;
    const float* cont = nullptr;
    int64_t ldc = 0;
    hipEvent_t ev_p1_begin = nullptr, ev_p1_end = nullptr, ev_p2_begin = nullptr, ev_p2_end = nullptr;
};

size_t lsm_part1_tiles(int64_t M);
hipError_t lsm_fold_table(hipStream_t st, double* cK, int N, double c0, double g);
inline void gbm_fold_constants(double S0, double K, double r, double sigma, double T, int n_steps, double* c0, double* g)
{
    const double dt = T / n_steps, L2E = 1.4426950408889634074;
    const float a = (float)((r - 0.5 * sigma * sigma) * dt * L2E);
    const float s0 = (float)S0;
    *c0 = (double)s0 * (double)s0 / K;
    *g = std::exp2(2.0 * (double)a);
}
hipError_t lsm_finalize(hipStream_t st, const double* part, const double* gmom, double* result,
                        int nblk, int N);

hipError_t lsm_step(hipStream_t st, const LsmProblem& p, const LsmWorkspace& w, int semantics,
                    int t, bool external_moments);
hipError_t lsm_reduce_step_moments(hipStream_t st, const LsmWorkspace& w, int t, int nblk);
int lsm_step_blocks(int64_t M);
int lsm_sweep_blocks(int64_t M);
int lsm_step_block_threads();
size_t lsm_sweep_args_bytes();
void lsm_sweep_args_image(const LsmProblem& p, const LsmWorkspace& w, int semantics, bool fill_state, void* out,
                          bool external_moments = false);
int lsm_multi_groups(int64_t M, int K, int device_cus);
hipError_t lsm_step_multi(hipStream_t st, const void* table_dev, int K, int G, int semantics, bool vec4, int N, int t);
hipError_t lsm_reduce_step_moments_multi(hipStream_t st, const void* table_dev, int K, int t);
hipError_t lsm_final_multi(hipStream_t st, const void* table_dev, int K, int64_t M);
hipError_t lsm_sweep_indirect(hipStream_t st, const LsmProblem& p, const LsmWorkspace& w, int semantics,
                              const void* args_dev);

hipError_t lsm_pass1_moments(hipStream_t st, const LsmProblem& p, const LsmWorkspace& w);
hipError_t lsm_pass2_apply(hipStream_t st, const LsmProblem& p, const LsmWorkspace& w,
                           bool write_state, bool solve_from_moments = false);

hipError_t lsm_final_reduce(hipStream_t st, const LsmProblem& p, const LsmWorkspace& w, int tval,
                            bool use_flags = false, bool fill_state = false);

constexpr int kMlpPartialStride2 = 4800;
constexpr int kMlpPartialStride3 = 8960;
constexpr int kMlpMaxGroups = 256;
constexpr int kMlpQ16MaxRows = 4096;
struct MlpTrainPlan {
    const float* data;
    float* params;
    float* adam_m;
    float* adam_v;
    float* partial;
    double* loss_acc;
    int64_t nrows, batch, first_step;
    int hidden, layers;
    float* wt;
    double lr, beta1, beta2, eps, weight_decay, dropout;
    uint64_t seed;
    uint64_t shuffle_key;
    bool wt_current = false;
    bool allow_q16 = false;
    const int64_t* step_off = nullptr;
    int64_t rows_global = 0;
    const uint32_t* drop_pos = nullptr;
    double* gred = nullptr;
    int (*allreduce)(void* user, double* dptr, int count) = nullptr;
    void* allreduce_user = nullptr;
};
struct MlpBatchJob {
    const float* data;
    int64_t nrows, batch, first_step;
    float *params, *adam_m, *adam_v, *partial, *wt;
    double* loss_acc;
    double lr;
    uint64_t seed, shuffle_key;
    const double* nrows_dev = nullptr;
    bool allow_q16 = false;
};
size_t mlp_batch_table_bytes(int n);
bool mlp_batch_supported(int hidden, int layers, int64_t batch);
void mlp_batch_table_image(const MlpBatchJob* jobs, int n, int hidden, int layers, double beta1, double beta2, double eps,
                           double weight_decay, double dropout, void* out);
hipError_t mlp_train_epoch_batch(hipStream_t st, const void* table_dev, int n, int hidden, int layers, int64_t max_steps,
                                 int max_tiles32, int max_tiles16, const double* bc1_dev, const double* bc2_dev);
int64_t mlp_q16_rows(int hidden);
hipError_t mlp_train_step_batch(hipStream_t st, const void* table_dev, int n, int hidden, int grid_tiles, int step_base,
                                const double* bc1_dev, const double* bc2_dev, const int* tile_prefix_dev = nullptr);
hipError_t mlp_tile_prefix(hipStream_t st, const void* table_dev, int n, int* prefix_dev);
size_t mlp_partial_bytes(int hidden, int layers, int64_t batch);
size_t mlp_wt_bytes(int hidden, int layers);
int mlp_train_param_count(int hidden, int layers);
int mlp_train_kernel_choice(int hidden, int layers, int64_t batch);
hipError_t mlp_dropout_masks(hipStream_t st, int variant, int hidden, int layers, int64_t n_rows, const uint32_t* keys,
                             uint32_t step, uint64_t seed, double dropout, uint8_t* out);
int mlp_apply_param_count(int hidden, int layers);
hipError_t mlp_apply_pass2(hipStream_t st, const LsmProblem& p, int hidden, int layers, const float* params,
                           const double* feat_mean, const double* feat_std, double y_mean, double y_std,
                           double dropout, uint64_t seed, float* sx, int32_t* tex, int64_t col_base0, int64_t col_base1);
int localvol_param_count(int hidden, int layers);
hipError_t localvol_paths(hipStream_t st, float* S, int64_t ld, int64_t M, int N, int layers, const float* params,
                          const float* Z, double S0, double r, double T, double K, double m_scale,
                          double tau_scale, double eps_out);
constexpr int kOls7Stats = 36;
size_t ols7_scratch_bytes(int64_t M, int N);
hipError_t ols7_comoments(hipStream_t st, const LsmProblem& p, const double* D, void* scratch, const double** stats_dev);
hipError_t ols7_pass2(hipStream_t st, const LsmProblem& p, const double* feat_mean, const double* feat_std,
                      const double* w7, double y_mean, double y_std, float* sx, int32_t* tex);
size_t nn_rows_scratch_bytes(int64_t M, int N);
hipError_t nn_rows_count(hipStream_t st, const LsmProblem& p, const double* D, void* scratch, const int64_t** total_dev,
                         const double** stats_dev);
hipError_t nn_rows_write(hipStream_t st, const LsmProblem& p, const double* D, void* scratch, const double* feat_mean,
                         const double* feat_std, double y_mean, double y_std, float* data, int64_t cap);
size_t nn_stats_scratch_bytes();
hipError_t nn_feature_stats(hipStream_t st, const double* x, const int32_t* t, const double* y, int64_t n,
                            double T, double dt, double* scratch, double* out16);
hipError_t mlp_shuffle_indices(hipStream_t st, int64_t n, uint64_t shuffle_key, int64_t* out);
hipError_t nn_scan_counts(hipStream_t st, const int32_t* cnt, int64_t n, int64_t* offs);
hipError_t nn_rows_half_counts(hipStream_t st, const LsmProblem& p, int64_t half, int64_t* counts_dev);
size_t mlp_shard_scratch_bytes(int64_t rows_global);
hipError_t mlp_shard_select(hipStream_t st, int64_t rows_global, uint64_t shuffle_key, const int64_t* gstart,
                            const int64_t* lstart, int nseg, int group ,
                            void* scratch, int64_t* sel_row, int64_t* sel_i, const int64_t** total_dev);
hipError_t mlp_shard_gather(hipStream_t st, const float* data, const int64_t* sel_row, const int64_t* sel_i,
                            int64_t n_local, int64_t batch, int64_t steps, float* data_epoch, uint32_t* drop_pos,
                            int64_t* step_off);
hipError_t mlp_train_steps(hipStream_t st, const MlpTrainPlan& t);
int64_t mlp_plan_kernel_batch(const MlpTrainPlan& t);

int cn_padded_width(int hidden);
size_t cn_scratch_bytes(int64_t M);
const double* cn_header(const LsmProblem& p, void* scratch);
hipError_t cn_count(hipStream_t st, const LsmProblem& p, const LsmWorkspace& w, void* scratch, int t, double Dt);
hipError_t cn_rows(hipStream_t st, const LsmProblem& p, const LsmWorkspace& w, void* scratch, int t, double Dt,
                   float* data);
hipError_t cn_init(hipStream_t st, int hidden, int t, uint64_t seed, float* params, float* m, float* v);
hipError_t cn_forward(hipStream_t st, const LsmProblem& p, const LsmWorkspace& w, void* scratch, int t, double Dt,
                      int hidden, const float* params, float* cont);

}
```

### options_model_amd/csrc/omc_lsm.hip

```cpp
#include "omc_lsm_dev.h"

#include <cstdlib>
#include <cstring>

namespace omc {

template <int SEM, int VEC, int BLOCK>
__global__ __launch_bounds__(BLOCK) void lsm_step_kernel(StepArgs a)
{
    lsm_step_body<SEM, VEC, BLOCK>(a, blockIdx.x, a.nblk);
}

template <int SEM, int VEC, int BLOCK>
__global__ __launch_bounds__(BLOCK) void lsm_step_ind_kernel(const StepArgs* __restrict__ ap, int t)
{
    StepArgs a = *ap;
    a.t = t;
    lsm_step_body<SEM, VEC, BLOCK>(a, blockIdx.x, a.nblk);
}

__global__ __launch_bounds__(kBlock) void lsm_reduce_step_kernel(const double* part, double* gmom, int t,
                                                                 int nblk, int pstride, int gstride)
{
    lsm_reduce_step_body(part, gmom, t, nblk, pstride, gstride);
}

template <int VEC, int TPW, int PUT>
__global__ __launch_bounds__(kBlock) void lsm_pass1_kernel(Pass1Args a) { lsm_pass1_body<VEC, TPW, PUT>(a); }

__global__ __launch_bounds__(kBlock) void lsm_reduce_pass1_kernel(const double* part1, double* gmom,
                                                                  int64_t ntiles, int N)
{
    lsm_reduce_pass1_body(part1, gmom, ntiles, N);
}

template <int VEC, bool WRITE_STATE>
__global__ __launch_bounds__(kBlock) void lsm_pass2_kernel(Pass2Args a) { lsm_pass2_body<VEC, WRITE_STATE>(a); }

template <int VEC, int TPW, int PUT>
__global__ __launch_bounds__(kBlock) void lsm_pass1_fold_kernel(Pass1Args a) { lsm_pass1_fold_body<VEC, TPW, PUT>(a); }
template <int VEC, int PUT>
__global__ __launch_bounds__(kBlock) void lsm_pass2_fold_kernel(Pass2Args a) { lsm_pass2_fold_body<VEC, PUT>(a); }

__global__ void lsm_fold_table_kernel(double* __restrict__ cK, int N, double c0, double g)
{
    if (threadIdx.x != 0 || blockIdx.x != 0) return;
    double c = c0;
    cK[0] = c;
    for (int t = 1; t <= N; ++t) {
        c *= g;
        cK[t] = c;
    }
}

template <int VEC>
__global__ __launch_bounds__(kBlock) void lsm_final_kernel(FinalArgs a) { lsm_final_body<VEC>(a); }

template <int VEC>
__global__ __launch_bounds__(kBlock) void lsm_final_ind_kernel(const FinalArgs* __restrict__ ap)
{
    lsm_final_body<VEC>(*ap);
}

__global__ __launch_bounds__(kBlock) void lsm_finalize_kernel(const double* part, const double* gmom,
                                                              double* result, int nblk, int N, int pstride)
{
    lsm_finalize_body(part, gmom, result, nblk, N, pstride);
}

struct FinalizeArgs {
    const double* part;
    const double* gmom;
    double* result;
    int nblk, N, pstride, gstride;
};
struct SweepArgs {
    StepArgs step;
    FinalArgs fin;
    FinalizeArgs fz;
};

__global__ __launch_bounds__(kBlock) void lsm_finalize_ind_kernel(const FinalizeArgs* __restrict__ ap)
{
    const FinalizeArgs a = *ap;
    lsm_finalize_body(a.part, a.gmom, a.result, a.nblk, a.N, a.pstride, a.gstride);
}

template <int SEM, int VEC, int BLOCK>
__global__ __launch_bounds__(BLOCK) void lsm_step_multi_kernel(const SweepArgs* __restrict__ tab, int G, int t)
{
    const int k = (int)blockIdx.x / G;
    StepArgs a = tab[k].step;
    a.t = t;
    lsm_step_body<SEM, VEC, BLOCK>(a, (int)blockIdx.x - k * G, G);
}

__global__ __launch_bounds__(kBlock) void lsm_reduce_step_multi_kernel(const SweepArgs* __restrict__ tab, int t)
{
    const StepArgs& a = tab[blockIdx.x].step;
    lsm_reduce_step_body(a.part, a.gmom, t, a.nblk, a.pstride, a.gstride);
}

template <int VEC>
__global__ __launch_bounds__(kBlock) void lsm_final_multi_kernel(const SweepArgs* __restrict__ tab)
{
    lsm_final_body<VEC>(tab[blockIdx.z].fin);
}

__global__ __launch_bounds__(kBlock) void lsm_finalize_multi_kernel(const SweepArgs* __restrict__ tab)
{
    const FinalizeArgs a = tab[blockIdx.x].fz;
    lsm_finalize_body(a.part, a.gmom, a.result, a.nblk, a.N, a.pstride, a.gstride);
}

static inline bool vec4_ok(const LsmProblem& p)
{
    return (p.M % 4) == 0 && (p.ld % 4) == 0 && ((uintptr_t)p.S % 16) == 0;
}

int lsm_step_blocks(int64_t M)
{
    const int64_t per_block = (int64_t)kBlock * 4;
    int64_t b = (M + per_block - 1) / per_block;
    if (b < 1) b = 1;
    return (int)(b > kMaxLsmBlocks ? kMaxLsmBlocks : b);
}

int lsm_step_block_threads()
{
    static const int v = [] {
        const char* e = getenv("OMC_STEP_BLOCK");
        const int x = e ? atoi(e) : 0;
        return x == 512 ? 512 : 1024;
    }();
    return v;
}

int lsm_sweep_blocks(int64_t M)
{
    const int64_t per_block = (int64_t)lsm_step_block_threads() * 4;
    int64_t b = (M + per_block - 1) / per_block;
    if (b < 1) b = 1;
    return (int)(b > kStepMaxBlocks ? kStepMaxBlocks : b);
}

size_t lsm_part1_tiles(int64_t M)
{
    return (size_t)((M + kBlock - 1) / kBlock);
}

static void fill_step_args(StepArgs& a, const LsmProblem& p, const LsmWorkspace& w, int t, bool external_moments)
{
    a.S = p.S; a.ld = p.ld; a.M = p.M; a.N = p.N; a.is_put = p.is_put;
    a.K = p.K; a.invK = 1.0 / p.K;
    a.sx = w.sx; a.tex = w.tex; a.live = w.live; a.D = w.D; a.part = w.part; a.gmom = w.gmom; a.betas = w.betas;
    a.t = t; a.nblk = lsm_sweep_blocks(p.M); a.external = external_moments ? 1 : 0;
    a.pstride = kPStride;
    a.gstride = w.gstride;
    a.cont = w.cont; a.ldc = w.ldc;
}

template <int SEM, int VEC, int BLOCK>
static void launch_step(hipStream_t st, const StepArgs& a, const StepArgs* ind, int t, size_t dyn)
{
    const dim3 grid(a.nblk), block(BLOCK);
    if (ind) hipLaunchKernelGGL((lsm_step_ind_kernel<SEM, VEC, BLOCK>), grid, block, dyn, st, ind, t);
    else hipLaunchKernelGGL((lsm_step_kernel<SEM, VEC, BLOCK>), grid, block, dyn, st, a);
}

static hipError_t lsm_step_impl(hipStream_t st, const LsmProblem& p, const LsmWorkspace& w, int semantics,
                                int t, bool external_moments, const StepArgs* ind)
{
    StepArgs a;
    fill_step_args(a, p, w, t, external_moments);
    const bool v4 = vec4_ok(p);
    const size_t dyn = semantics == 1 ? sizeof(double) * (size_t)(p.N + 1) : 0;
    const bool big = lsm_step_block_threads() == 1024;
#define OMC_STEP(SEM, VEC)                                                       \
    do {                                                                         \
        if (big) launch_step<SEM, VEC, 1024>(st, a, ind, t, dyn);               \
        else launch_step<SEM, VEC, 512>(st, a, ind, t, dyn);                    \
    } while (0)
    if (semantics == 0) {
        if (v4) OMC_STEP(0, 4); else OMC_STEP(0, 1);
    } else {
        if (v4) OMC_STEP(1, 4); else OMC_STEP(1, 1);
    }
#undef OMC_STEP
    return hipGetLastError();
}

hipError_t lsm_step(hipStream_t st, const LsmProblem& p, const LsmWorkspace& w, int semantics,
                    int t, bool external_moments)
{
    return lsm_step_impl(st, p, w, semantics, t, external_moments, nullptr);
// ... 45 lines not shown
        else hipLaunchKernelGGL((lsm_step_multi_kernel<SEM, VEC, 512>), grid, dim3(512), dyn, st, tab, G, t);  \
    } while (0)
    if (semantics == 0) {
        if (vec4) OMC_STEPM(0, 4); else OMC_STEPM(0, 1);
    } else {
        if (vec4) OMC_STEPM(1, 4); else OMC_STEPM(1, 1);
    }
#undef OMC_STEPM
    return hipGetLastError();
}

hipError_t lsm_reduce_step_moments_multi(hipStream_t st, const void* table_dev, int K, int t)
{
    hipLaunchKernelGGL(lsm_reduce_step_multi_kernel, dim3(K), dim3(kBlock), 0, st, (const SweepArgs*)table_dev, t);
    return hipGetLastError();
}

hipError_t lsm_final_multi(hipStream_t st, const void* table_dev, int K, int64_t M)
{
    const SweepArgs* tab = (const SweepArgs*)table_dev;
    const int nblk = lsm_step_blocks(M);
    if ((M % 4) == 0) hipLaunchKernelGGL((lsm_final_multi_kernel<4>), dim3(nblk, 1, K), dim3(kBlock), 0, st, tab);
    else hipLaunchKernelGGL((lsm_final_multi_kernel<1>), dim3(nblk, 1, K), dim3(kBlock), 0, st, tab);
    hipLaunchKernelGGL(lsm_finalize_multi_kernel, dim3(K), dim3(kBlock), 0, st, tab);
    return hipGetLastError();
}

hipError_t lsm_sweep_indirect(hipStream_t st, const LsmProblem& p, const LsmWorkspace& w, int semantics,
                              const void* args_dev)
{
    const SweepArgs* sa = (const SweepArgs*)args_dev;
    for (int t = p.N; t >= 1; --t) {
        hipError_t e = lsm_step_impl(st, p, w, semantics, t, false, &sa->step);
        if (e != hipSuccess) return e;
    }
    const int nblk = lsm_step_blocks(p.M);
    if ((p.M % 4) == 0) hipLaunchKernelGGL((lsm_final_ind_kernel<4>), dim3(nblk), dim3(kBlock), 0, st, &sa->fin);
    else hipLaunchKernelGGL((lsm_final_ind_kernel<1>), dim3(nblk), dim3(kBlock), 0, st, &sa->fin);
    hipLaunchKernelGGL(lsm_finalize_ind_kernel, dim3(1), dim3(kBlock), 0, st, &sa->fz);
    return hipGetLastError();
}

hipError_t lsm_reduce_step_moments(hipStream_t st, const LsmWorkspace& w, int t, int nblk)
{
    hipLaunchKernelGGL(lsm_reduce_step_kernel, dim3(1), dim3(kBlock), 0, st, w.part, w.gmom, t, nblk,
                       kPStride, w.gstride);
    return hipGetLastError();
}

hipError_t lsm_fold_table(hipStream_t st, double* cK, int N, double c0, double g)
{
    hipLaunchKernelGGL(lsm_fold_table_kernel, dim3(1), dim3(64), 0, st, cK, N, c0, g);
    return hipGetLastError();
}

static hipError_t lsm_pass1_moments_fold(hipStream_t st, const LsmProblem& p, const LsmWorkspace& w)
{
    Pass1Args a;
    const int64_t P = p.M / 2;
    a.S = p.S; a.ld = p.ld; a.M = P; a.N = p.N; a.is_put = p.is_put;
    a.K = p.K; a.invK = 1.0 / p.K; a.D = w.D; a.part1 = w.part1; a.cK = p.fold_cK;
    const bool v4 = (P % 4) == 0 && (p.ld % 4) == 0 && ((uintptr_t)p.S % 16) == 0;
    static const int tpw_env = getenv("OMC_FOLD_TPW") ? atoi(getenv("OMC_FOLD_TPW")) : 0;
    const int tpw = (v4 && (tpw_env == 1 || tpw_env == 4)) ? tpw_env : 2;
    const int64_t per_wave = 64 * (int64_t)(v4 ? 4 : 1) * tpw;
    a.ntiles = (P + per_wave - 1) / per_wave;
    static const int tch_env = getenv("OMC_PASS1_TCHUNK") ? atoi(getenv("OMC_PASS1_TCHUNK")) : 0;
    const int64_t wgs_x = (a.ntiles + 3) / 4;
    a.tchunk = (tch_env >= 2 && tch_env <= kFoldMaxChunk) ? tch_env : 32;
    const dim3 grid((unsigned)wgs_x, (unsigned)((p.N - 1 + a.tchunk - 1) / a.tchunk));
    if (w.ev_p1_begin) (void)hipEventRecord(w.ev_p1_begin, st);
    if (v4 && tpw == 1) {
        if (p.is_put) hipLaunchKernelGGL((lsm_pass1_fold_kernel<4, 1, 1>), grid, dim3(kBlock), 0, st, a);
        else hipLaunchKernelGGL((lsm_pass1_fold_kernel<4, 1, 0>), grid, dim3(kBlock), 0, st, a);
    } else if (v4 && tpw == 4) {
        if (p.is_put) hipLaunchKernelGGL((lsm_pass1_fold_kernel<4, 4, 1>), grid, dim3(kBlock), 0, st, a);
        else hipLaunchKernelGGL((lsm_pass1_fold_kernel<4, 4, 0>), grid, dim3(kBlock), 0, st, a);
    } else if (v4) {
        if (p.is_put) hipLaunchKernelGGL((lsm_pass1_fold_kernel<4, 2, 1>), grid, dim3(kBlock), 0, st, a);
        else hipLaunchKernelGGL((lsm_pass1_fold_kernel<4, 2, 0>), grid, dim3(kBlock), 0, st, a);
    } else {
        if (p.is_put) hipLaunchKernelGGL((lsm_pass1_fold_kernel<1, 2, 1>), grid, dim3(kBlock), 0, st, a);
        else hipLaunchKernelGGL((lsm_pass1_fold_kernel<1, 2, 0>), grid, dim3(kBlock), 0, st, a);
    }
    if (w.ev_p1_end) (void)hipEventRecord(w.ev_p1_end, st);
    hipLaunchKernelGGL(lsm_reduce_pass1_kernel, dim3(p.N - 1), dim3(kBlock), 0, st, w.part1, w.gmom, a.ntiles, p.N);
    return hipGetLastError();
}

hipError_t lsm_pass1_moments(hipStream_t st, const LsmProblem& p, const LsmWorkspace& w)
{
    if (p.N < 2) return hipSuccess;
    if (p.fold_cK) return lsm_pass1_moments_fold(st, p, w);
    Pass1Args a;
    a.S = p.S; a.ld = p.ld; a.M = p.M; a.N = p.N; a.is_put = p.is_put;
    a.K = p.K; a.invK = 1.0 / p.K; a.D = w.D; a.part1 = w.part1;
    const bool v4 = vec4_ok(p);
    static const int tpw_env = getenv("OMC_PASS1_TPW") ? atoi(getenv("OMC_PASS1_TPW")) : 0;
    static const int tch_env = getenv("OMC_PASS1_TCHUNK") ? atoi(getenv("OMC_PASS1_TCHUNK")) : 0;
    const int tpw = (v4 && (tpw_env == 1 || tpw_env == 2 || tpw_env == 8)) ? tpw_env : 4;
    const int64_t per_wave = 64 * (int64_t)(v4 ? 4 : 1) * tpw;
    a.ntiles = (p.M + per_wave - 1) / per_wave;
    static const int cus = [] {
        int dev = 0, n = 0;
        if (hipGetDevice(&dev) != hipSuccess || hipDeviceGetAttribute(&n, hipDeviceAttributeMultiprocessorCount, dev) != hipSuccess)
            n = 256;
        return n > 0 ? n : 256;
    }();
    int tchunk = 32;
    const int64_t wgs_x = (a.ntiles + 3) / 4;
    if (wgs_x <= 3 * (int64_t)cus && p.N > 2) {
        const int chunks = (int)((3 * (int64_t)cus) / wgs_x);
        const int t = (p.N - 1 + chunks - 1) / chunks;
        if (t <= 126 && t >= 32) tchunk = t;
    }
    a.tchunk = (tch_env >= 2 && tch_env <= kPass1MaxChunk) ? tch_env : tchunk;
    const dim3 grid((unsigned)((a.ntiles + 3) / 4), (unsigned)((p.N - 1 + a.tchunk - 1) / a.tchunk));
    if (w.ev_p1_begin) (void)hipEventRecord(w.ev_p1_begin, st);
    auto launch = [&](auto vec, auto tp) {
        constexpr int V = decltype(vec)::value, T = decltype(tp)::value;
        if (p.is_put) hipLaunchKernelGGL((lsm_pass1_kernel<V, T, 1>), grid, dim3(kBlock), 0, st, a);
        else hipLaunchKernelGGL((lsm_pass1_kernel<V, T, 0>), grid, dim3(kBlock), 0, st, a);
    };
    using std::integral_constant;
    if (!v4) launch(integral_constant<int, 1>{}, integral_constant<int, 4>{});
    else if (tpw == 1) launch(integral_constant<int, 4>{}, integral_constant<int, 1>{});
    else if (tpw == 2) launch(integral_constant<int, 4>{}, integral_constant<int, 2>{});
    else if (tpw == 8) launch(integral_constant<int, 4>{}, integral_constant<int, 8>{});
    else launch(integral_constant<int, 4>{}, integral_constant<int, 4>{});
    if (w.ev_p1_end) (void)hipEventRecord(w.ev_p1_end, st);
    hipLaunchKernelGGL(lsm_reduce_pass1_kernel, dim3(p.N - 1), dim3(kBlock), 0, st, w.part1, w.gmom,
                       a.ntiles, p.N);
    return hipGetLastError();
}

hipError_t lsm_pass2_apply(hipStream_t st, const LsmProblem& p, const LsmWorkspace& w,
                           bool write_state, bool solve_from_moments)
{
    Pass2Args a;
    a.S = p.S; a.ld = p.ld; a.M = p.M; a.N = p.N; a.is_put = p.is_put;
    a.K = p.K; a.invK = 1.0 / p.K; a.D = w.D; a.betas = w.betas; a.sx = w.sx; a.tex = w.tex;
    a.part = w.part;
    if (solve_from_moments) {
        a.gmom = w.gmom;
        a.betas_out = w.betas;
    }
    static const int fvec_env = getenv("OMC_FOLD_P2_VEC") ? atoi(getenv("OMC_FOLD_P2_VEC")) : 0;
    const int fvec = (fvec_env == 1 || fvec_env == 2 || fvec_env == 4) ? fvec_env : ((p.M / 2) >= (int64_t(1) << 21) ? 4 : 2);
    const int nblk = lsm_step_blocks(p.fold_cK ? (p.M / 2) * (4 / fvec) : p.M);
    a.nblk = nblk; a.pstride = kPStride;
    const size_t dyn = sizeof(double) * 4 * (size_t)(p.N + 1);
    const bool v4 = vec4_ok(p);
    if (w.ev_p2_begin) (void)hipEventRecord(w.ev_p2_begin, st);
    if (p.fold_cK) {
        if (write_state) return hipErrorInvalidValue;
        a.M = p.M / 2;
        a.cK = p.fold_cK;
        const bool f4 = (a.M % 4) == 0 && (p.ld % 4) == 0 && ((uintptr_t)p.S % 16) == 0;
        auto launch = [&](auto vec) {
            constexpr int V = decltype(vec)::value;
            if (p.is_put) hipLaunchKernelGGL((lsm_pass2_fold_kernel<V, 1>), dim3(nblk), dim3(kBlock), dyn, st, a);
            else hipLaunchKernelGGL((lsm_pass2_fold_kernel<V, 0>), dim3(nblk), dim3(kBlock), dyn, st, a);
        };
        if (f4 && fvec == 4) launch(std::integral_constant<int, 4>{});
        else if (f4 && fvec == 2) launch(std::integral_constant<int, 2>{});
        else launch(std::integral_constant<int, 1>{});
    } else if (v4) {
        if (write_state) hipLaunchKernelGGL((lsm_pass2_kernel<4, true>), dim3(nblk), dim3(kBlock), dyn, st, a);
        else hipLaunchKernelGGL((lsm_pass2_kernel<4, false>), dim3(nblk), dim3(kBlock), dyn, st, a);
    } else {
        if (write_state) hipLaunchKernelGGL((lsm_pass2_kernel<1, true>), dim3(nblk), dim3(kBlock), dyn, st, a);
        else hipLaunchKernelGGL((lsm_pass2_kernel<1, false>), dim3(nblk), dim3(kBlock), dyn, st, a);
    }
    if (w.ev_p2_end) (void)hipEventRecord(w.ev_p2_end, st);
    hipLaunchKernelGGL(lsm_finalize_kernel, dim3(1), dim3(kBlock), 0, st, w.part, w.gmom, w.result,
                       nblk, p.N, kPStride);
    return hipGetLastError();
}

hipError_t lsm_finalize(hipStream_t st, const double* part, const double* gmom, double* result,
                        int nblk, int N)
{
    hipLaunchKernelGGL(lsm_finalize_kernel, dim3(1), dim3(kBlock), 0, st, part, gmom, result, nblk, N,
                       kPStride);
    return hipGetLastError();
}

hipError_t lsm_final_reduce(hipStream_t st, const LsmProblem& p, const LsmWorkspace& w, int tval, bool use_flags,
                            bool fill_state)
{
    FinalArgs a;
    fill_final_args(a, p, w, tval, use_flags, fill_state);
    const int nblk = a.nblk;
    if ((p.M % 4) == 0) hipLaunchKernelGGL((lsm_final_kernel<4>), dim3(nblk), dim3(kBlock), 0, st, a);
    else hipLaunchKernelGGL((lsm_final_kernel<1>), dim3(nblk), dim3(kBlock), 0, st, a);
    hipLaunchKernelGGL(lsm_finalize_kernel, dim3(1), dim3(kBlock), 0, st, w.part, w.gmom, w.result,
                       nblk, p.N, kPStride);
    return hipGetLastError();
}

}
```

### options_model_amd/csrc/omc_lsm_dev.h

```cpp
#pragma once
#include "omc_device.h"
#include "omc_kernels.h"
#include <type_traits>

namespace omc {


constexpr int kPStride = kMaxLsmBlocks;

template <int VEC>
__device__ __forceinline__ void loadf(const float* __restrict__ p, float (&v)[VEC])
{
    if constexpr (VEC == 4) {
        const float4 x = *reinterpret_cast<const float4*>(p);
        v[0] = x.x; v[1] = x.y; v[2] = x.z; v[3] = x.w;
    } else if constexpr (VEC == 2) {
        const float2 x = *reinterpret_cast<const float2*>(p);
        v[0] = x.x; v[1] = x.y;
    } else {
        static_assert(VEC == 1, "loadf: 1, 2 or 4 floats");
        v[0] = *p;
    }
}
template <int VEC>
__device__ __forceinline__ void loadf_stream(const float* __restrict__ p, float (&v)[VEC])
{
    if constexpr (VEC == 4) {
        typedef float f4 __attribute__((ext_vector_type(4)));
        const f4 x = __builtin_nontemporal_load(reinterpret_cast<const f4*>(p));
        v[0] = x.x; v[1] = x.y; v[2] = x.z; v[3] = x.w;
    } else if constexpr (VEC == 2) {
        typedef float f2 __attribute__((ext_vector_type(2)));
        const f2 x = __builtin_nontemporal_load(reinterpret_cast<const f2*>(p));
        v[0] = x.x; v[1] = x.y;
    } else {
        static_assert(VEC == 1, "loadf_stream: 1, 2 or 4 floats");
        v[0] = __builtin_nontemporal_load(p);
    }
}
template <int VEC>
__device__ __forceinline__ void loadi(const int32_t* __restrict__ p, int32_t (&v)[VEC])
{
    if constexpr (VEC == 4) {
        const int4 x = *reinterpret_cast<const int4*>(p);
        v[0] = x.x; v[1] = x.y; v[2] = x.z; v[3] = x.w;
    } else {
        v[0] = *p;
    }
}
template <int VEC>
__device__ __forceinline__ void storef(float* p, const float (&v)[VEC])
{
    if constexpr (VEC == 4) *reinterpret_cast<float4*>(p) = make_float4(v[0], v[1], v[2], v[3]);
    else *p = v[0];
}
template <int VEC>
__device__ __forceinline__ void storei(int32_t* p, const int32_t (&v)[VEC])
{
    if constexpr (VEC == 4) *reinterpret_cast<int4*>(p) = make_int4(v[0], v[1], v[2], v[3]);
    else *p = v[0];
}

struct StepArgs {
    const float* S;
    int64_t ld, M;
    int N, is_put;
    double K, invK;
    float* sx;
    int32_t* tex;
    float* live;
    const double* D;
    double* part;
    double* gmom;
    double* betas;
    int t, nblk, external;
    int pstride;
    int gstride;
    const float* cont;
    int64_t ldc;
};

constexpr int kStepMaxBlocks = 256;
constexpr int kStepPL = kStepMaxBlocks / 64;
constexpr int kStepMaxItems = 32;

template <int SEM, int VEC, int BLOCK>
__device__ __forceinline__ void lsm_step_body(StepArgs a, const int w, const int G)
{
    constexpr int WAVES = BLOCK / 64;
    __shared__ double wl[WAVES * kWaveRedDoubles];
    __shared__ double sh_w[kStepMaxItems * WAVES * 8];
    __shared__ double sh_beta[4];
    extern __shared__ double sh_D[];

    const int tid = threadIdx.x, lane = tid & 63, wave = tid >> 6;
    const int t = a.t, N = a.N;
    if (w >= a.nblk || t > N) return;
    const bool do_apply = t < N, do_mom = t >= 2, init = (t == N);
    const bool values = a.cont != nullptr;
    const float* controw = values ? a.cont + (int64_t)t * a.ldc : nullptr;

    if (SEM == 1 && do_mom) {
        for (int k = tid; k <= N; k += BLOCK) sh_D[k] = a.D[k];
    }

    const bool pro = do_apply && wave == 0 && !values;
    double pv[kStepPL][8];
    if (pro && !a.external) {
        const double* pp = a.part + (size_t)(t & 1) * 8 * a.pstride;
#pragma unroll
        for (int i = 0; i < kStepPL; ++i) {
            const int b = lane + 64 * i;
            const bool ok = b < a.nblk;
            const double* p = pp + (ok ? b : 0);
#pragma unroll
            for (int q = 0; q < 8; ++q) {
                const double v = p[(size_t)q * a.pstride];
                pv[i][q] = ok ? v : 0.0;
            }
        }
    }
    __builtin_amdgcn_sched_barrier(0);

    const float* St = a.S + (int64_t)t * a.ld;
    const float* Sm = St - a.ld;
    const int64_t stride = (int64_t)a.nblk * BLOCK * VEC;
    struct Chunk {
        float st[VEC], sm[VEC], sx[VEC];
        int32_t tex[VEC];
        uint32_t exw;
        int64_t j;
    };
    auto load_chunk = [&](Chunk& c) {
        loadf<VEC>(St + c.j, c.st);
        if (do_mom) loadf<VEC>(Sm + c.j, c.sm);
        if (!init) {
            if (SEM == 0) {
                loadf<VEC>(a.live + c.j, c.sx);
            } else {
                loadf<VEC>(a.sx + c.j, c.sx);
                loadi<VEC>(a.tex + c.j, c.tex);
            }
        }
    };
    auto slot_chunks = [&](int vb) { return (int)((a.M - (int64_t)vb * BLOCK * VEC + stride - 1) / stride); };
    int cur_vb = w, cur_i = 0, cur_n = slot_chunks(w);
    auto fetch = [&](Chunk& c, bool& valid, bool& last) {
        valid = cur_vb < a.nblk;
        last = false;
        if (!valid) return;
        c.j = ((int64_t)cur_vb * BLOCK + tid) * VEC + (int64_t)cur_i * stride;
        if (c.j < a.M) load_chunk(c);
        last = cur_i + 1 == cur_n;
        if (last) {
            cur_vb += G;
// ... 375 lines not shown
    load_rows(bufB, min(t0 + 1, tl));
    __builtin_amdgcn_sched_barrier(0);
#pragma unroll
    for (int k = 0; k < TPW; ++k) {
#pragma unroll
        for (int v = 0; v < VEC; ++v) {
            const double pa = payoff_d(sn[k][v], K, is_put), pb = fold_pay(fold_u(cKN, sn[k][v]), K, is_put);
            pNA[k][v] = (valid[k] && pa > 0.0) ? pa : 0.0;
            pNB[k][v] = (valid[k] && pb > 0.0) ? pb : 0.0;
        }
    }
    const float thr = itm_threshold(K, is_put);
    float thrk[TPW];
#pragma unroll
    for (int k = 0; k < TPW; ++k) thrk[k] = valid[k] ? thr : (is_put ? -__builtin_inff() : __builtin_inff());
    unsigned long long vmask[TPW];
#pragma unroll
    for (int k = 0; k < TPW; ++k) vmask[k] = __builtin_amdgcn_ballot_w64(valid[k]);
    auto process = [&](auto put_tag, const float (&buf)[TPW][VEC], int t) {
        constexpr bool IS_PUT = decltype(put_tag)::value;
        double acc[8];
#pragma unroll
        for (int q = 0; q < 8; ++q) acc[q] = 0.0;
        int cnt = 0;
        const double ck = shC[wave][t - t0];
        auto add_row = [&](double u, double y, double m) {
            const double u2 = u * u;
            acc[1] += u;
            acc[2] += u2;
            acc[3] = fma(u2, u, acc[3]);
            acc[4] = fma(u2, u2, acc[4]);
            acc[5] = fma(y, m, acc[5]);
            acc[6] = fma(u, y, acc[6]);
            acc[7] = fma(u2, y, acc[7]);
        };
#pragma unroll
        for (int k = 0; k < TPW; ++k) {
#pragma unroll
            for (int v = 0; v < VEC; ++v) {
                const float sf = buf[k][v];
                const double ua = fma((double)sf, invK, -1.0);
                const double ub = fold_u(ck, sf);
                const bool ia = IS_PUT ? sf < thrk[k] : sf > thrk[k];
                const bool ibc = IS_PUT ? ub < 0.0 : ub > 0.0;
                const unsigned long long ma = __builtin_amdgcn_ballot_w64(ia);
                const unsigned long long mb = __builtin_amdgcn_ballot_w64(ibc) & vmask[k];
                const bool ib = valid[k] && ibc;
                cnt += __builtin_popcountll(ma | mb);
                const double mp = (ia || ib) ? 1.0 : 0.0;
                add_row((ia ? ua : ub) * mp, ia ? pNA[k][v] : pNB[k][v], mp);
                const unsigned long long bb = ma & mb;
                if (bb != 0) {
                    asm volatile("; a lane with both partners in the money" ::);
                    cnt += __builtin_popcountll(bb);
                    const bool both = ia && ib;
                    const double ms = both ? 1.0 : 0.0;
                    add_row(ub * ms, pNB[k][v], ms);
                }
            }
        }
        const double d = shD[wave][t - t0];
        acc[0] = lane == 0 ? (double)cnt : 0.0;
        acc[5] *= d;
        acc[6] *= d;
        acc[7] *= d;
        const double s = wave_reduce8(acc, wl[wave]);
        if ((lane & 7) == 0) a.part1[((size_t)t * a.ntiles + tg) * 8 + (lane >> 3)] = s;
    };
    auto sweep = [&](auto put_tag) {
        for (int t = t0; t < t1; t += 3) {
            load_rows(bufC, min(t + 2, tl));
            __builtin_amdgcn_sched_barrier(0);
            process(put_tag, bufA, t);
            if (t + 1 < t1) {
                load_rows(bufA, min(t + 3, tl));
                __builtin_amdgcn_sched_barrier(0);
                process(put_tag, bufB, t + 1);
            }
            if (t + 2 < t1) {
                load_rows(bufB, min(t + 4, tl));
                __builtin_amdgcn_sched_barrier(0);
                process(put_tag, bufC, t + 2);
            }
        }
    };
    if (PUT == 1 || (PUT < 0 && is_put))
        sweep(std::true_type{});
    else
        sweep(std::false_type{});
}

__device__ __forceinline__ void lsm_reduce_pass1_body(const double* __restrict__ part1,
                                                      double* __restrict__ gmom, int64_t ntiles,
                                                      int N)
{
    if ((int)blockIdx.x + 1 >= N) return;
    __shared__ double sh[kBlock / 64][8];
    const int tid = threadIdx.x;
    const int t = blockIdx.x + 1;
    const double2* pp = reinterpret_cast<const double2*>(part1 + (size_t)t * ntiles * 8);
    double s[8];
#pragma unroll
    for (int q = 0; q < 8; ++q) s[q] = 0.0;
    for (int64_t i = tid; i < ntiles; i += kBlock) {
        double2 r[4];
#pragma unroll
        for (int k = 0; k < 4; ++k) r[k] = pp[i * 4 + k];
#pragma unroll
        for (int k = 0; k < 4; ++k) {
            s[2 * k] += r[k].x;
            s[2 * k + 1] += r[k].y;
        }
    }
#pragma unroll
    for (int q = 0; q < 8; ++q) {
#pragma unroll
        for (int off = 32; off >= 1; off >>= 1) s[q] += __shfl_xor(s[q], off);
    }
    if ((tid & 63) == 0) {
#pragma unroll
        for (int q = 0; q < 8; ++q) sh[tid >> 6][q] = s[q];
    }
    __syncthreads();
    if (tid < 8) gmom[(size_t)t * 8 + tid] = (sh[0][tid] + sh[1][tid]) + (sh[2][tid] + sh[3][tid]);
}

__device__ __forceinline__ void lsm_solve_all_body(const double* __restrict__ gmom, double* __restrict__ betas,
                                     int N)
{
    const int t = blockIdx.x * blockDim.x + threadIdx.x;
    if (t < 1 || t >= N) return;
    double m[8], beta[3];
#pragma unroll
    for (int q = 0; q < 8; ++q) m[q] = gmom[(size_t)t * 8 + q];
    solve_poly2(m, beta);
    double* bo = betas + (size_t)t * 4;
    bo[0] = beta[0]; bo[1] = beta[1]; bo[2] = beta[2]; bo[3] = m[0];
}

struct Pass2Args {
    const float* S;
    int64_t ld, M;
    int N, is_put;
    double K, invK;
    const double* D;
    const double* betas;
    float* sx;
    int32_t* tex;
    double* part;
    int nblk, pstride;
    const double* gmom = nullptr;
    double* betas_out = nullptr;
    const double* cK = nullptr;
};

template <int VEC, bool WRITE_STATE>
__device__ __forceinline__ void lsm_pass2_body(Pass2Args a)
{
    if ((int)blockIdx.x >= a.nblk) return;
    __shared__ double red[kNQ * kRedStride];
    extern __shared__ double sh_b[];
    const int tid = threadIdx.x;
    const int N = a.N;
    if (a.gmom) {
        for (int t = tid; t <= N; t += kBlock) {
            double m[8], beta[3] = {0.0, 0.0, 0.0};
            const bool inner = t >= 1 && t < N;
#pragma unroll
            for (int q = 0; q < 8; ++q) m[q] = inner ? a.gmom[(size_t)t * 8 + q] : 0.0;
            if (inner) solve_poly2(m, beta);
            const bool fit = inner && m[0] > 0.5;
            sh_b[4 * t] = fit ? beta[0] : __builtin_huge_val();
            sh_b[4 * t + 1] = fit ? beta[1] : 0.0;
            sh_b[4 * t + 2] = fit ? beta[2] : 0.0;
            sh_b[4 * t + 3] = 0.0;
            if (blockIdx.x == 0 && inner && a.betas_out) {
                double* bo = a.betas_out + (size_t)t * 4;
                bo[0] = beta[0]; bo[1] = beta[1]; bo[2] = beta[2]; bo[3] = m[0];
            }
        }
    } else {
        for (int k = tid; k < (N + 1) * 4; k += kBlock) {
            const int t = k >> 2;
            const bool fit = t >= 1 && t < N && a.betas[(size_t)t * 4 + 3] > 0.5;
            sh_b[k] = fit ? a.betas[k] : ((k & 3) == 0 ? __builtin_huge_val() : 0.0);
        }
    }
    __syncthreads();
    const double K = a.K, invK = a.invK;
    const int is_put = a.is_put;
    double acc[8];
#pragma unroll
    for (int q = 0; q < 8; ++q) acc[q] = 0.0;
    const int64_t stride = (int64_t)a.nblk * kBlock * VEC;
    for (int64_t j = ((int64_t)blockIdx.x * kBlock + tid) * VEC; j < a.M; j += stride) {
        float sx[VEC];
        int32_t tex[VEC];
        loadf<VEC>(a.S + (int64_t)N * a.ld + j, sx);
#pragma unroll
        for (int v = 0; v < VEC; ++v) tex[v] = N;
        auto decide = [&](const float (&row)[VEC], int t) {
            const double b0 = sh_b[4 * t], b1 = sh_b[4 * t + 1], b2 = sh_b[4 * t + 2];
#pragma unroll
            for (int v = 0; v < VEC; ++v) {
                const double sd = (double)row[v];
                const double imm = is_put ? K - sd : sd - K;
                const double u = fma(sd, invK, -1.0);
                const double cont = fma(u, fma(u, b2, b1), b0);
                const bool ex = (tex[v] == N) & (imm > 0.0) & (imm > cont);
                sx[v] = ex ? row[v] : sx[v];
                tex[v] = ex ? t : tex[v];
            }
        };
        auto live = [&]() {
            bool l = false;
#pragma unroll
            for (int v = 0; v < VEC; ++v) l |= (tex[v] == N);
            return l;
        };
        constexpr int U = 8;
        int t = N - 1;
        const float* col = a.S + j;
        for (; t >= U && live(); t -= U) {
            float st[U][VEC];
#pragma unroll
            for (int k = 0; k < U; ++k) loadf_stream<VEC>(col + (int64_t)(t - k) * a.ld, st[k]);
#pragma unroll
            for (int k = 0; k < U; ++k) decide(st[k], t - k);
        }
        for (; t >= 1 && live(); --t) {
            float st[VEC];
            loadf_stream<VEC>(col + (int64_t)t * a.ld, st);
            decide(st, t);
        }
#pragma unroll
        for (int v = 0; v < VEC; ++v) {
            double p = payoff_d(sx[v], K, is_put);
            p = p > 0.0 ? p : 0.0;
            const double cf = p * a.D[tex[v] - 1];
            acc[0] += cf;
            acc[1] += cf * cf;
            acc[2] += (tex[v] < N) ? 1.0 : 0.0;
            acc[3] += (cf == 0.0) ? 1.0 : 0.0;
        }
        if (WRITE_STATE) {
            storef<VEC>(a.sx + j, sx);
            storei<VEC>(a.tex + j, tex);
        }
    }
    const double s = block_reduce8(acc, red);
    if (tid < 64 && (tid & 7) == 0) a.part[(size_t)(tid >> 3) * a.pstride + blockIdx.x] = s;
}

template <int VEC, int PUT = -1>
__device__ __forceinline__ void lsm_pass2_fold_body(Pass2Args a)
{
    if ((int)blockIdx.x >= a.nblk) return;
    __shared__ double red[kNQ * kRedStride];
    extern __shared__ double sh_b[];
    const int tid = threadIdx.x;
    const int N = a.N;
    if (a.gmom) {
        for (int t = tid; t <= N; t += kBlock) {
            double m[8], beta[3] = {0.0, 0.0, 0.0};
            const bool inner = t >= 1 && t < N;
#pragma unroll
            for (int q = 0; q < 8; ++q) m[q] = inner ? a.gmom[(size_t)t * 8 + q] : 0.0;
            if (inner) solve_poly2(m, beta);
            const bool fit = inner && m[0] > 0.5;
            sh_b[4 * t] = fit ? beta[0] : __builtin_huge_val();
            sh_b[4 * t + 1] = fit ? beta[1] : 0.0;
            sh_b[4 * t + 2] = fit ? beta[2] : 0.0;
            sh_b[4 * t + 3] = a.cK[t];
            if (blockIdx.x == 0 && inner && a.betas_out) {
                double* bo = a.betas_out + (size_t)t * 4;
                bo[0] = beta[0]; bo[1] = beta[1]; bo[2] = beta[2]; bo[3] = m[0];
            }
        }
    } else {
        for (int k = tid; k < (N + 1) * 4; k += kBlock) {
            const int t = k >> 2;
            const bool fit = t >= 1 && t < N && a.betas[(size_t)t * 4 + 3] > 0.5;
            sh_b[k] = (k & 3) == 3 ? a.cK[t] : (fit ? a.betas[k] : ((k & 3) == 0 ? __builtin_huge_val() : 0.0));
        }
    }
    __syncthreads();
    const double K = a.K, invK = a.invK;
    const int is_put = PUT < 0 ? a.is_put : PUT;
    double acc[8];
#pragma unroll
    for (int q = 0; q < 8; ++q) acc[q] = 0.0;
    const int64_t stride = (int64_t)a.nblk * kBlock * VEC;
    for (int64_t j = ((int64_t)blockIdx.x * kBlock + tid) * VEC; j < a.M; j += stride) {
        float sxa[VEC], sxb[VEC];
        int32_t texa[VEC], texb[VEC];
        loadf<VEC>(a.S + (int64_t)N * a.ld + j, sxa);
#pragma unroll
        for (int v = 0; v < VEC; ++v) {
            sxb[v] = sxa[v];
            texa[v] = texb[v] = N;
        }
        auto decide = [&](const float (&row)[VEC], int t) {
            const double b0 = sh_b[4 * t], b1 = sh_b[4 * t + 1], b2 = sh_b[4 * t + 2], ck = sh_b[4 * t + 3];
#pragma unroll
            for (int v = 0; v < VEC; ++v) {
                const double sd = (double)row[v];
                const double imm = is_put ? K - sd : sd - K;
                const double u = fma(sd, invK, -1.0);
                const double cont = fma(u, fma(u, b2, b1), b0);
                const bool ex = (texa[v] == N) & (imm > 0.0) & (imm > cont);
                sxa[v] = ex ? row[v] : sxa[v];
                texa[v] = ex ? t : texa[v];
                const double ub = fold_u(ck, row[v]);
                const double immb = fold_pay(ub, K, is_put);
                const double contb = fma(ub, fma(ub, b2, b1), b0);
                const bool exb = (texb[v] == N) & (immb > 0.0) & (immb > contb);
                sxb[v] = exb ? row[v] : sxb[v];
                texb[v] = exb ? t : texb[v];
            }
        };
        auto live = [&]() {
            bool l = false;
#pragma unroll
            for (int v = 0; v < VEC; ++v) l |= (texa[v] == N) | (texb[v] == N);
            return l;
        };
        constexpr int U = 8;
        int t = N - 1;
        const float* col = a.S + j;
        auto fetch = [&](float (&b)[U][VEC], int tt) {
#pragma unroll
            for (int k = 0; k < U; ++k) loadf_stream<VEC>(col + (int64_t)max(tt - k, 1) * a.ld, b[k]);
        };
        auto work = [&](const float (&b)[U][VEC], int tt) {
#pragma unroll
            for (int k = 0; k < U; ++k)
                if (tt - k >= 1) decide(b[k], tt - k);
        };
        float bA[U][VEC], bB[U][VEC];
        if (t >= 1) fetch(bA, t);
        while (t >= 1 && live()) {
            if (t - U >= 1) fetch(bB, t - U);
            __builtin_amdgcn_sched_barrier(0);
            work(bA, t);
            t -= U;
            if (!(t >= 1 && live())) break;
            if (t - U >= 1) fetch(bA, t - U);
            __builtin_amdgcn_sched_barrier(0);
            work(bB, t);
            t -= U;
        }
#pragma unroll
        for (int v = 0; v < VEC; ++v) {
            double p = payoff_d(sxa[v], K, is_put);
            p = p > 0.0 ? p : 0.0;
            const double cf = p * a.D[texa[v] - 1];
            double pb = fold_pay(fold_u(sh_b[4 * texb[v] + 3], sxb[v]), K, is_put);
            pb = pb > 0.0 ? pb : 0.0;
            const double cfb = pb * a.D[texb[v] - 1];
            acc[0] += cf;
            acc[1] += cf * cf;
            acc[2] += (texa[v] < N) ? 1.0 : 0.0;
            acc[3] += (cf == 0.0) ? 1.0 : 0.0;
            acc[0] += cfb;
            acc[1] += cfb * cfb;
            acc[2] += (texb[v] < N) ? 1.0 : 0.0;
            acc[3] += (cfb == 0.0) ? 1.0 : 0.0;
        }
    }
    const double s = block_reduce8(acc, red);
    if (tid < 64 && (tid & 7) == 0) a.part[(size_t)(tid >> 3) * a.pstride + blockIdx.x] = s;
}

struct FinalArgs {
    float* sx;
    int32_t* tex;
    const float* live;
    int64_t M;
    int N, is_put, tval, fill_state;
    double K;
    const double* D;
    double* part;
    int nblk, pstride;
};

template <int VEC>
__device__ __forceinline__ void lsm_final_body(FinalArgs a)
{
    if ((int)blockIdx.x >= a.nblk) return;
    __shared__ double red[kNQ * kRedStride];
    const int tid = threadIdx.x;
    double acc[8];
#pragma unroll
    for (int q = 0; q < 8; ++q) acc[q] = 0.0;
    const int64_t stride = (int64_t)a.nblk * kBlock * VEC;
    for (int64_t j = ((int64_t)blockIdx.x * kBlock + tid) * VEC; j < a.M; j += stride) {
        float sx[VEC];
        int32_t tex[VEC];
        loadf<VEC>(a.sx + j, sx);
        loadi<VEC>(a.tex + j, tex);
        if (a.live) {
            float sn[VEC];
            loadf<VEC>(a.live + j, sn);
            bool any = false;
#pragma unroll
            for (int v = 0; v < VEC; ++v) {
                if (!(sn[v] < 0.0f)) { sx[v] = sn[v]; tex[v] = a.N; any = true; }
            }
            if (a.fill_state && any) {
                storef<VEC>(a.sx + j, sx);
                storei<VEC>(a.tex + j, tex);
            }
        }
#pragma unroll
        for (int v = 0; v < VEC; ++v) {
            double p = payoff_d(sx[v], a.K, a.is_put);
            p = p > 0.0 ? p : 0.0;
            const double cf = p * a.D[tex[v] - a.tval];
            acc[0] += cf;
            acc[1] += cf * cf;
            acc[2] += (tex[v] < a.N) ? 1.0 : 0.0;
            acc[3] += (cf == 0.0) ? 1.0 : 0.0;
        }
    }
    const double s = block_reduce8(acc, red);
    if (tid < 64 && (tid & 7) == 0) a.part[(size_t)(tid >> 3) * a.pstride + blockIdx.x] = s;
}

__device__ __forceinline__ void lsm_finalize_body(const double* __restrict__ part,
                                                  const double* __restrict__ gmom,
                                                  double* __restrict__ result, int nblk, int N,
                                                  int pstride, int gstride = 8)
{
    __shared__ double red[kNQ * kRedStride];
    const int tid = threadIdx.x;
    double acc[8];
#pragma unroll
    for (int q = 0; q < 8; ++q) acc[q] = 0.0;
    for (int i = tid; i < nblk; i += kBlock) {
#pragma unroll
        for (int q = 0; q < 4; ++q) acc[q] += part[(size_t)q * pstride + i];
    }
    for (int t = 1 + tid; t < N; t += kBlock) acc[4] += gmom[(size_t)t * gstride];
    const double s = block_reduce8(acc, red);
    if (tid < 64 && (tid & 7) == 0) result[tid >> 3] = s;
}

}
```

Before: 639.5 billion.

## Precompute per-step exercise intervals in float bit space for pass-2 fold

Adds a per-step kernel that turns each fitted quadratic continuation value into at most two intervals of float bit patterns where exercise holds, for both the direct and the antithetic-folded path. It finds these by solving for the roots analytically and then checking the region around each root with wave-ballot probes. The pass-2 sweep then decides exercise with integer range compares instead of several f64 FMAs per element per step. Steps whose pattern is irregular fall back to the f64 path. This costs an extra small kernel launch and adds correctness risk if an interval is built wrong; a debug check API is included to verify the tables.

```diff
diff --git a/include/omc.h b/include/omc.h
--- a/include/omc.h
+++ b/include/omc.h
@@ -8,7 +8,7 @@
 extern "C" {
 #endif
 
-#define OMC_ABI_VERSION 10
+#define OMC_ABI_VERSION 11
 
 typedef struct omc_ctx omc_ctx;
 
@@ -126,6 +126,8 @@
 } omc_greeks;
 int omc_price_american_greeks(omc_ctx* ctx, const omc_params* p, double bump, const double* betas, double* betas_out,
                               omc_greeks* out);
+int omc_pass2_tables_check(omc_ctx* ctx, int is_put, double K, int n_steps, const double* betas, const double* cK,
+                           int irregular_every, int64_t* mismatches, int* irregular);
 int omc_price_european(omc_ctx* ctx, const omc_params* p, omc_result* res);
 
 int omc_heston_price_strikes(omc_ctx* ctx, int64_t n_paths, int n_steps, double S0, double r,
diff --git a/options_model_amd/_build.py b/options_model_amd/_build.py
--- a/options_model_amd/_build.py
+++ b/options_model_amd/_build.py
@@ -11,7 +11,7 @@
 LIB = os.path.join(LIBDIR, "libomc.so")
 SOURCES = ["omc_paths.hip", "omc_lsm.hip", "omc_batch.hip", "omc_mlp.hip", "omc_contnet.hip", "omc_rows.hip", "omc_ols7.hip", "omc_greeks.hip", "omc_comm.hip", "omc_p2p.hip",
            "omc_api.hip"]
-HEADERS = ["omc_device.h", "omc_kernels.h", "omc_lsm_dev.h", "omc_paths_dev.h", "omc_contnet_dev.h", "omc_batch.h", "omc_greeks.h", "omc_comm.h", "omc_p2p.h",
+HEADERS = ["omc_device.h", "omc_crit.h", "omc_kernels.h", "omc_lsm_dev.h", "omc_paths_dev.h", "omc_contnet_dev.h", "omc_batch.h", "omc_greeks.h", "omc_comm.h", "omc_p2p.h",
            os.path.join("..", "..", "include", "omc.h")]
 ARCH = "gfx950"
 FLAGS_STAMP = os.path.join(LIBDIR, "libomc.flags")
diff --git a/options_model_amd/_ffi.py b/options_model_amd/_ffi.py
--- a/options_model_amd/_ffi.py
+++ b/options_model_amd/_ffi.py
@@ -8,7 +8,7 @@
 
 from . import _build
 
-ABI_VERSION = 10
+ABI_VERSION = 11
 
 SEMANTICS = {"reference": 0, "textbook": 1, "two_pass": 2}
 MODELS = {"gbm": 0, "heston": 1}
@@ -100,6 +100,7 @@
     "omc_p2p_status": (C.c_int, [_P, C.POINTER(C.c_int), C.POINTER(C.c_int), C.POINTER(C.c_uint64)]),
     "omc_price_american": (C.c_int, [_P, C.POINTER(Params), C.POINTER(Result), _P, _I64]),
     "omc_price_american_greeks": (C.c_int, [_P, C.POINTER(Params), _D, _P, _P, C.POINTER(Greeks)]),
+    "omc_pass2_tables_check": (C.c_int, [_P, _I, _D, _I, _P, _P, _I, _P, _P]),
     "omc_price_european": (C.c_int, [_P, C.POINTER(Params), C.POINTER(Result)]),
     "omc_heston_price_strikes": (C.c_int, [_P, _I64, _I] + [_D] * 8 + [_U64, _U64, _I, _P, _I, _I, _P, _P]),
     "omc_heston_price_surface": (C.c_int, [_P, _I64, _I] + [_D] * 7 + [_U64, _I, _P, _P, _I, _P, _P, _I, _I, _P, _P]),
@@ -503,6 +504,19 @@
             keep_paths.shape[1] if keep_paths else 0))
         return res.as_dict()
 
+    def pass2_tables_check(self, is_put, K, betas, cK, irregular_every=0):
+        b = np.ascontiguousarray(betas, np.float64)
+        ck = np.ascontiguousarray(cK, np.float64)
+        N = b.shape[0] - 1
+        if b.shape != (N + 1, 4) or ck.shape != (N + 1,):
+            raise ValueError("betas must be [N+1][4] and cK [N+1].")
+        mism = np.zeros((N + 1, 2), np.int64)
+        irr = np.zeros(N + 1, np.int32)
+        _check(self.lib, self.lib.omc_pass2_tables_check(self.handle, int(bool(is_put)), float(K), N, b.ctypes.data,
+                                                         ck.ctypes.data, int(irregular_every), mism.ctypes.data,
+                                                         irr.ctypes.data))
+        return mism, irr.astype(bool)
+
     def price_american_greeks(self, params: Params, bump=0.01, betas=None, want_betas=False):
         N = int(params.n_steps)
         b = None
diff --git a/options_model_amd/csrc/omc_api.hip b/options_model_amd/csrc/omc_api.hip
--- a/options_model_amd/csrc/omc_api.hip
+++ b/options_model_amd/csrc/omc_api.hip
@@ -99,7 +99,7 @@
     int device = 0;
     hipStream_t stream = nullptr;
     bool own_stream = false;
-    DevBuf S, sx, tex, ex, D, part, gmom, betas, part1, result, scratch, sweep_args;
+    DevBuf S, sx, tex, ex, D, part, gmom, betas, part1, result, scratch, sweep_args, crit;
     DevBuf bslab, btable, bres, bdisc;
     DevBuf mlp_part, mlp_loss, mlp_wt;
     DevBuf mlp_gred, shard;
@@ -131,6 +131,8 @@
     int seq_step_wgs = 0;
     int gbm_vec = 0, heston_vec = 0;
     int fold = 1;
+    int pass2_tables = 1;
+    int pass2_irr_every = 0;
     DevBuf foldC;
     DevBuf gk_part, gk_res;
     struct FoldKey { int N = -1; double c0 = 0, g = 0; } fold_key[2];
@@ -238,6 +240,12 @@
     if ((rc = c->result.ensure(sizeof(double) * 8))) return rc;
     w->part1 = nullptr;
     w->part1_tiles = 0;
+    w->crit = nullptr;
+    if (two_pass && c->pass2_tables) {
+        if ((rc = c->crit.ensure(sizeof(uint32_t) * 8 * (size_t)(N + 1)))) return rc;
+        w->crit = (uint32_t*)c->crit.p;
+    }
+    w->crit_irr_every = c->pass2_irr_every;
     if (two_pass) {
         const size_t tiles = omc::lsm_part1_tiles(M);
         if ((rc = c->part1.ensure(sizeof(double) * 8 * (size_t)(N + 1) * tiles))) return rc;
@@ -533,7 +541,7 @@
     for (DevBuf* b : {&c->S, &c->sx, &c->tex, &c->ex, &c->D, &c->part, &c->gmom, &c->betas, &c->part1,
                       &c->result, &c->scratch, &c->sweep_args, &c->bslab, &c->btable, &c->bres, &c->bdisc,
                       &c->mlp_part, &c->mlp_loss, &c->mlp_wt, &c->mlp_gred, &c->shard, &c->S2, &c->seq_local, &c->part1b, &c->gmomb, &c->seq_vote, &c->cn_scratch, &c->cn_data, &c->cn_net, &c->cn_cont,
-                      &c->mS, &c->mstate, &c->mtable, &c->mb_slab, &c->mb_table, &c->mb_bc})
+                      &c->mS, &c->mstate, &c->mtable, &c->mb_slab, &c->mb_table, &c->mb_bc, &c->crit})
         b->release();
     if (c->sweep_pin) (void)hipHostFree(c->sweep_pin);
     if (c->mtab_pin) (void)hipHostFree(c->mtab_pin);
@@ -626,6 +634,8 @@
     if (!strcmp(key, "gbm_vec")) c->gbm_vec = (int)value;
     else if (!strcmp(key, "alloc_limit")) g_alloc_limit = value > 0 ? (size_t)value : 0;
     else if (!strcmp(key, "fold_antithetic")) c->fold = value <= 0 ? 0 : (value >= 2 ? 2 : 1);
+    else if (!strcmp(key, "pass2_tables")) c->pass2_tables = value ? 1 : 0;
+    else if (!strcmp(key, "pass2_tables_irregular_every")) c->pass2_irr_every = value > 0 ? (int)value : 0;
     else if (!strcmp(key, "heston_vec")) c->heston_vec = (int)value;
     else if (!strcmp(key, "world_size")) c->world = value > 0 ? (int)value : 1;
     else if (!strcmp(key, "step_graph")) c->step_graph = value < 0 ? -1 : (value ? 1 : 0);
@@ -1119,6 +1129,31 @@
                 c->distributed() ? c->world : 1);
     res->folded = (!S_keep && fold_applies(c, p)) ? 1 : 0;
     return read_kernel_times(c->ev, p, res);
+}
+
+int omc_pass2_tables_check(omc_ctx* c, int is_put, double K, int n_steps, const double* betas, const double* cK,
+                           int irregular_every, int64_t* mismatches, int* irregular)
+{
+    if (!c || !betas || !cK || !mismatches || !irregular) return fail(-7, "null pointer.");
+    if (n_steps < 1 || n_steps > omc::kMaxSteps || !(K > 0.0)) return fail(-4, "invalid n_steps or strike.");
+    HIP_TRY(hipSetDevice(c->device));
+    const size_t n1 = (size_t)n_steps + 1;
+    const size_t o_cK = sizeof(double) * 4 * n1, o_tab = o_cK + sizeof(double) * n1, o_mism = o_tab + sizeof(uint32_t) * 8 * n1,
+                 bytes = o_mism + sizeof(unsigned long long) * 2 * n1;
+    int rc;
+    if ((rc = c->scratch.ensure(bytes))) return rc;
+    char* b = (char*)c->scratch.p;
+    HIP_TRY(hipMemcpyAsync(b, betas, sizeof(double) * 4 * n1, hipMemcpyHostToDevice, c->stream));
+    HIP_TRY(hipMemcpyAsync(b + o_cK, cK, sizeof(double) * n1, hipMemcpyHostToDevice, c->stream));
+    HIP_TRY(hipMemsetAsync(b + o_mism, 0, sizeof(unsigned long long) * 2 * n1, c->stream));
+    HIP_TRY(omc::lsm_crit_check(c->stream, (const double*)b, (const double*)(b + o_cK), (uint32_t*)(b + o_tab), n_steps,
+                                is_put ? 1 : 0, K, irregular_every, (unsigned long long*)(b + o_mism)));
+    std::vector<uint32_t> tab(8 * n1);
+    HIP_TRY(hipMemcpyAsync(tab.data(), b + o_tab, sizeof(uint32_t) * 8 * n1, hipMemcpyDeviceToHost, c->stream));
+    HIP_TRY(hipMemcpyAsync(mismatches, b + o_mism, sizeof(int64_t) * 2 * n1, hipMemcpyDeviceToHost, c->stream));
+    HIP_TRY(hipStreamSynchronize(c->stream));
+    for (size_t t = 0; t < n1; ++t) irregular[t] = tab[8 * t] == 0xffffffffu || tab[8 * t + 4] == 0xffffffffu;
+    return 0;
 }
 
 int omc_price_american_greeks(omc_ctx* c, const omc_params* p, double bump, const double* betas, double* betas_out,
diff --git a/options_model_amd/csrc/omc_crit.h b/options_model_amd/csrc/omc_crit.h
--- /dev/null
+++ b/options_model_amd/csrc/omc_crit.h
@@ -0,0 +1,159 @@
+#pragma once
+#include <stdint.h>
+#include <math.h>
+
+#if defined(__HIPCC__)
+#define OMC_HD __host__ __device__
+#else
+#define OMC_HD
+#endif
+
+namespace omc {
+
+constexpr uint32_t kCritTop = 0x7f800000u;
+constexpr int kCritHalf = 32;
+constexpr int kCritMaxCand = 6;
+
+struct CritIv {
+    uint32_t lo[2], len[2];
+};
+
+OMC_HD inline float crit_float(uint32_t o) { return __builtin_bit_cast(float, o); }
+OMC_HD inline uint32_t crit_bits(float f) { return __builtin_bit_cast(uint32_t, f); }
+
+template <class P, class O>
+OMC_HD inline uint64_t crit_mask64(const P& pred, const O& ord)
+{
+#if defined(__HIP_DEVICE_COMPILE__)
+    const int i = (int)(threadIdx.x & 63);
+    return __builtin_amdgcn_ballot_w64(pred(crit_float(ord(i))));
+#else
+    uint64_t m = 0;
+    for (int i = 0; i < 64; ++i) m |= (uint64_t)(pred(crit_float(ord(i))) ? 1 : 0) << i;
+    return m;
+#endif
+}
+
+OMC_HD inline int crit_candidates(int kind, int is_put, double K, double ck, double b0, double b1, double b2,
+                                  double (&cand)[kCritMaxCand])
+{
+    int n = 0;
+    auto add_u = [&](double u) {
+        double s;
+        if (kind == 0) s = K * (1.0 + u);
+        else s = (1.0 + u) > 0.0 ? ck / (1.0 + u) : -1.0;
+        if (s >= 0.0 && n < kCritMaxCand) cand[n++] = s;
+    };
+    cand[n++] = 0.0;
+    cand[n++] = __builtin_huge_val();
+    add_u(0.0);
+    if (b0 == __builtin_huge_val() && b1 == 0.0 && b2 == 0.0) return n;
+    if (!isfinite(b0) || !isfinite(b1) || !isfinite(b2)) return -1;
+    const double A = b2, B = b1 - (is_put ? -K : K), C = b0;
+    if (A == 0.0) {
+        if (fabs(B) <= 1e-9 * (fabs(b1) + K)) return -1;
+        add_u(-C / B);
+        return n;
+    }
+    const double disc = B * B - 4.0 * A * C;
+    const double scale = B * B + fabs(4.0 * A * C);
+    if (fabs(disc) <= 1e-9 * scale) return -1;
+    if (disc < 0.0) return n;
+    const double q = -0.5 * (B + copysign(sqrt(disc), B));
+    add_u(q / A);
+    if (q != 0.0) add_u(C / q);
+    return n;
+}
+
+template <class P>
+OMC_HD inline bool crit_build(const P& pred, const double* cand, int ncand, CritIv& out)
+{
+    out.lo[0] = out.lo[1] = out.len[0] = out.len[1] = 0;
+    uint32_t wa[kCritMaxCand], wb[kCritMaxCand];
+    int nw = 0;
+    for (int i = 0; i < ncand; ++i) {
+        const double s = cand[i];
+        const uint32_t o = s >= 3.4028234663852886e38 ? kCritTop : crit_bits((float)s);
+        const uint32_t a = o > (uint32_t)kCritHalf ? o - kCritHalf : 0u;
+        const uint32_t b = o + kCritHalf - 1 < kCritTop ? o + kCritHalf - 1 : kCritTop;
+        int k = nw++;
+        while (k > 0 && wa[k - 1] > a) {
+            wa[k] = wa[k - 1];
+            wb[k] = wb[k - 1];
+            --k;
+        }
+        wa[k] = a;
+        wb[k] = b;
+    }
+    int m = 0;
+    for (int i = 0; i < nw; ++i) {
+        if (m > 0 && wa[i] <= wb[m - 1] + 1) {
+            if (wb[i] > wb[m - 1]) wb[m - 1] = wb[i];
+        } else {
+            wa[m] = wa[i];
+            wb[m] = wb[i];
+            ++m;
+        }
+    }
+    nw = m;
+    int nint = 0;
+    bool cur = false, have = false;
+    uint32_t start = 0;
+    auto set = [&](bool v, uint32_t o) -> bool {
+        if (have && v == cur) return true;
+        if (v) start = o;
+        else if (have) {
+            if (nint == 2) return false;
+            out.lo[nint] = start;
+            out.len[nint] = o - start;
+            ++nint;
+        }
+        cur = v;
+        have = true;
+        return true;
+    };
+    uint32_t next = 0;
+    for (int w = 0; w <= nw; ++w) {
+        const uint32_t g0 = next, g1e = w < nw ? wa[w] : kCritTop + 1;
+        if (g1e > g0) {
+            const uint64_t span = (uint64_t)(g1e - 1 - g0);
+            const uint64_t mk = crit_mask64(pred, [&](int i) { return (uint32_t)(g0 + span * (uint64_t)i / 63u); });
+            if (mk != 0 && mk != ~0ull) return false;
+            const bool v = mk != 0;
+            if (have && v != cur) return false;
+            if (!set(v, g0)) return false;
+        }
+        if (w == nw) break;
+        int switches = 0;
+        for (uint32_t c0 = wa[w]; c0 <= wb[w]; c0 += 64) {
+            const uint32_t c1 = wb[w] - c0 >= 63 ? c0 + 63 : wb[w];
+            const int n = (int)(c1 - c0) + 1;
+            const uint64_t valid = n == 64 ? ~0ull : (1ull << n) - 1;
+            const uint64_t mk = crit_mask64(pred, [&](int i) { return c0 + (uint32_t)i <= c1 ? c0 + (uint32_t)i : c1; }) & valid;
+            const uint64_t prev = have ? (uint64_t)cur : (~mk & 1u);
+            uint64_t d = (mk ^ ((mk << 1) | prev)) & valid;
+            while (d) {
+                const int i = __builtin_ctzll(d);
+                d &= d - 1;
+                if (have && ++switches > ncand) return false;
+                if (!set((mk >> i) & 1u, c0 + (uint32_t)i)) return false;
+            }
+            if (c1 == wb[w]) break;
+        }
+        next = wb[w] + 1;
+    }
+    if (cur) {
+        if (nint == 2) return false;
+        out.lo[nint] = start;
+        out.len[nint] = kCritTop + 1 - start;
+        ++nint;
+    }
+    return true;
+}
+
+OMC_HD inline bool crit_in(const CritIv& t, uint32_t b)
+{
+    return (b - t.lo[0]) < t.len[0] || (b - t.lo[1]) < t.len[1];
+}
+
+}
diff --git a/options_model_amd/csrc/omc_kernels.h b/options_model_amd/csrc/omc_kernels.h
--- a/options_model_amd/csrc/omc_kernels.h
+++ b/options_model_amd/csrc/omc_kernels.h
@@ -84,6 +84,8 @@
     double* result;
     const float* cont = nullptr;
     int64_t ldc = 0;
+    uint32_t* crit = nullptr;
+    int crit_irr_every = 0;
     hipEvent_t ev_p1_begin = nullptr, ev_p1_end = nullptr, ev_p2_begin = nullptr, ev_p2_end = nullptr;
 };
 
@@ -119,6 +121,8 @@
 hipError_t lsm_pass1_moments(hipStream_t st, const LsmProblem& p, const LsmWorkspace& w);
 hipError_t lsm_pass2_apply(hipStream_t st, const LsmProblem& p, const LsmWorkspace& w,
                            bool write_state, bool solve_from_moments = false);
+hipError_t lsm_crit_check(hipStream_t st, const double* betas, const double* cK, uint32_t* tab, int N, int is_put,
+                          double K, int irr_every, unsigned long long* mism);
 
 hipError_t lsm_final_reduce(hipStream_t st, const LsmProblem& p, const LsmWorkspace& w, int tval,
                             bool use_flags = false, bool fill_state = false);
diff --git a/options_model_amd/csrc/omc_lsm.hip b/options_model_amd/csrc/omc_lsm.hip
--- a/options_model_amd/csrc/omc_lsm.hip
+++ b/options_model_amd/csrc/omc_lsm.hip
@@ -39,8 +39,16 @@
 
 template <int VEC, int TPW, int PUT>
 __global__ __launch_bounds__(kBlock) void lsm_pass1_fold_kernel(Pass1Args a) { lsm_pass1_fold_body<VEC, TPW, PUT>(a); }
-template <int VEC, int PUT>
-__global__ __launch_bounds__(kBlock) void lsm_pass2_fold_kernel(Pass2Args a) { lsm_pass2_fold_body<VEC, PUT>(a); }
+template <int VEC, int PUT, bool TAB>
+__global__ __launch_bounds__(kBlock) void lsm_pass2_fold_kernel(Pass2Args a) { lsm_pass2_fold_body<VEC, PUT, TAB>(a); }
+
+__global__ __launch_bounds__(128) void lsm_crit_build_kernel(CritArgs a) { lsm_crit_build_body(a); }
+__global__ __launch_bounds__(kBlock) void lsm_crit_check_kernel(const uint32_t* tab, const double* betas, const double* cK,
+                                                                int N, int is_put, double K, double invK,
+                                                                unsigned long long* mism)
+{
+    lsm_crit_check_body(tab, betas, cK, N, is_put, K, invK, mism);
+}
 
 __global__ void lsm_fold_table_kernel(double* __restrict__ cK, int N, double c0, double g)
 {
@@ -392,6 +400,16 @@
     const size_t dyn = sizeof(double) * 4 * (size_t)(p.N + 1);
     const bool v4 = vec4_ok(p);
     if (w.ev_p2_begin) (void)hipEventRecord(w.ev_p2_begin, st);
+    const bool tab = w.crit != nullptr && p.fold_cK != nullptr && !write_state;
+    if (tab) {
+        CritArgs c;
+        c.gmom = a.gmom; c.betas = w.betas; c.betas_out = a.betas_out; c.cK = p.fold_cK; c.tab = w.crit;
+        c.N = p.N; c.is_put = p.is_put; c.K = a.K; c.invK = a.invK; c.irr_every = w.crit_irr_every;
+        hipLaunchKernelGGL(lsm_crit_build_kernel, dim3(p.N + 1), dim3(128), 0, st, c);
+        a.gmom = nullptr;
+        a.betas_out = nullptr;
+        a.crit = w.crit;
+    }
     if (p.fold_cK) {
         if (write_state) return hipErrorInvalidValue;
         a.M = p.M / 2;
@@ -399,8 +417,13 @@
         const bool f4 = (a.M % 4) == 0 && (p.ld % 4) == 0 && ((uintptr_t)p.S % 16) == 0;
         auto launch = [&](auto vec) {
             constexpr int V = decltype(vec)::value;
-            if (p.is_put) hipLaunchKernelGGL((lsm_pass2_fold_kernel<V, 1>), dim3(nblk), dim3(kBlock), dyn, st, a);
-            else hipLaunchKernelGGL((lsm_pass2_fold_kernel<V, 0>), dim3(nblk), dim3(kBlock), dyn, st, a);
+            if (tab) {
+                if (p.is_put) hipLaunchKernelGGL((lsm_pass2_fold_kernel<V, 1, true>), dim3(nblk), dim3(kBlock), dyn, st, a);
+                else hipLaunchKernelGGL((lsm_pass2_fold_kernel<V, 0, true>), dim3(nblk), dim3(kBlock), dyn, st, a);
+            } else {
+                if (p.is_put) hipLaunchKernelGGL((lsm_pass2_fold_kernel<V, 1, false>), dim3(nblk), dim3(kBlock), dyn, st, a);
+                else hipLaunchKernelGGL((lsm_pass2_fold_kernel<V, 0, false>), dim3(nblk), dim3(kBlock), dyn, st, a);
+            }
         };
         if (f4 && fvec == 4) launch(std::integral_constant<int, 4>{});
         else if (f4 && fvec == 2) launch(std::integral_constant<int, 2>{});
@@ -418,6 +441,19 @@
     return hipGetLastError();
 }
 
+hipError_t lsm_crit_check(hipStream_t st, const double* betas, const double* cK, uint32_t* tab, int N, int is_put,
+                          double K, int irr_every, unsigned long long* mism)
+{
+    CritArgs c;
+    c.gmom = nullptr; c.betas = betas; c.betas_out = nullptr; c.cK = cK; c.tab = tab;
+    c.N = N; c.is_put = is_put; c.K = K; c.invK = 1.0 / K; c.irr_every = irr_every;
+    hipLaunchKernelGGL(lsm_crit_build_kernel, dim3(N + 1), dim3(128), 0, st, c);
+    if (N >= 2)
+        hipLaunchKernelGGL(lsm_crit_check_kernel, dim3(2048, N - 1), dim3(kBlock), 0, st, tab, betas, cK, N, is_put, K,
+                           c.invK, mism);
+    return hipGetLastError();
+}
+
 hipError_t lsm_finalize(hipStream_t st, const double* part, const double* gmom, double* result,
                         int nblk, int N)
 {
diff --git a/options_model_amd/csrc/omc_lsm_dev.h b/options_model_amd/csrc/omc_lsm_dev.h
--- a/options_model_amd/csrc/omc_lsm_dev.h
+++ b/options_model_amd/csrc/omc_lsm_dev.h
@@ -1,6 +1,7 @@
 #pragma once
 #include "omc_device.h"
 #include "omc_kernels.h"
+#include "omc_crit.h"
 #include <type_traits>
 
 namespace omc {
@@ -682,7 +683,144 @@
     const double* gmom = nullptr;
     double* betas_out = nullptr;
     const double* cK = nullptr;
+    const uint32_t* crit = nullptr;
 };
+
+struct CritStored {
+    double K, invK, b0, b1, b2;
+    int is_put;
+    __device__ bool operator()(float s) const
+    {
+        const double sd = (double)s;
+        const double imm = is_put ? K - sd : sd - K;
+        const double u = fma(sd, invK, -1.0);
+        const double cont = fma(u, fma(u, b2, b1), b0);
+        return (imm > 0.0) & (imm > cont);
+    }
+};
+struct CritPartner {
+    double K, ck, b0, b1, b2;
+    int is_put;
+    __device__ bool operator()(float s) const
+    {
+        const double ub = fold_u(ck, s);
+        const double immb = fold_pay(ub, K, is_put);
+        const double contb = fma(ub, fma(ub, b2, b1), b0);
+        return (immb > 0.0) & (immb > contb);
+    }
+};
+struct CritEither {
+    CritStored a;
+    CritPartner b;
+    int kind;
+    __device__ bool operator()(float s) const { return kind ? b(s) : a(s); }
+};
+constexpr uint32_t kCritIrregular = 0xffffffffu;
+
+struct CritArgs {
+    const double* gmom;
+    const double* betas;
+    double* betas_out;
+    const double* cK;
+    uint32_t* tab;
+    int N, is_put;
+    double K, invK;
+    int irr_every = 0;
+};
+
+__device__ __forceinline__ void lsm_crit_build_body(CritArgs a)
+{
+    const int t = (int)blockIdx.x, kind = (int)(threadIdx.x >> 6), lane = (int)(threadIdx.x & 63);
+    const int N = a.N;
+    const bool inner = t >= 1 && t < N;
+    double beta[3] = {0.0, 0.0, 0.0};
+    bool fit = false;
+    if (a.gmom) {
+        double m[8];
+#pragma unroll
+        for (int q = 0; q < 8; ++q) m[q] = inner ? a.gmom[(size_t)t * 8 + q] : 0.0;
+        if (inner) solve_poly2(m, beta);
+        fit = inner && m[0] > 0.5;
+        if (inner && kind == 0 && lane == 0 && a.betas_out) {
+            double* bo = a.betas_out + (size_t)t * 4;
+            bo[0] = beta[0]; bo[1] = beta[1]; bo[2] = beta[2]; bo[3] = m[0];
+        }
+    } else if (inner) {
+        fit = a.betas[(size_t)t * 4 + 3] > 0.5;
+        if (fit) {
+            beta[0] = a.betas[(size_t)t * 4];
+            beta[1] = a.betas[(size_t)t * 4 + 1];
+            beta[2] = a.betas[(size_t)t * 4 + 2];
+        }
+    }
+    const double b0 = fit ? beta[0] : __builtin_huge_val(), b1 = fit ? beta[1] : 0.0, b2 = fit ? beta[2] : 0.0;
+    CritIv iv;
+    iv.lo[0] = iv.lo[1] = iv.len[0] = iv.len[1] = 0;
+    if (inner && (kind == 0 || a.cK)) {
+        const double ck = kind ? a.cK[t] : 0.0;
+        double cand[kCritMaxCand];
+        const int n = crit_candidates(kind, a.is_put, a.K, ck, b0, b1, b2, cand);
+        bool ok = n >= 0 && !(a.irr_every > 0 && t % a.irr_every == 0);
+        if (ok) ok = crit_build(CritEither{CritStored{a.K, a.invK, b0, b1, b2, a.is_put},
+                                           CritPartner{a.K, ck, b0, b1, b2, a.is_put}, kind}, cand, n, iv);
+        if (!ok) {
+            iv.lo[0] = kCritIrregular;
+            iv.lo[1] = iv.len[0] = iv.len[1] = 0;
+        }
+    }
+    if (lane == 0) {
+        uint32_t* o = a.tab + (size_t)t * 8 + 4 * kind;
+        o[0] = iv.lo[0]; o[1] = iv.lo[1]; o[2] = iv.len[0]; o[3] = iv.len[1];
+    }
+}
+
+__device__ __forceinline__ bool crit_load_tables(const uint32_t* __restrict__ tab, uint32_t* sh_t, int N)
+{
+    int irr = 0;
+    for (int t = threadIdx.x; t <= N; t += kBlock) {
+        const uint4 x = *reinterpret_cast<const uint4*>(tab + (size_t)t * 8);
+        const uint4 y = *reinterpret_cast<const uint4*>(tab + (size_t)t * 8 + 4);
+        const bool bad = x.x == kCritIrregular || y.x == kCritIrregular;
+        irr |= bad;
+        *reinterpret_cast<uint4*>(sh_t + 8 * t) = make_uint4(bad ? kCritIrregular : x.x, x.y, x.z, x.w);
+        *reinterpret_cast<uint4*>(sh_t + 8 * t + 4) = y;
+    }
+    return __syncthreads_or(irr) != 0;
+}
+
+__device__ __forceinline__ void crit_fits(const double* __restrict__ betas, int t, int N, double& b0, double& b1,
+                                          double& b2)
+{
+    const bool fit = t >= 1 && t < N && betas[(size_t)t * 4 + 3] > 0.5;
+    b0 = fit ? betas[(size_t)t * 4] : __builtin_huge_val();
+    b1 = fit ? betas[(size_t)t * 4 + 1] : 0.0;
+    b2 = fit ? betas[(size_t)t * 4 + 2] : 0.0;
+}
+
+__device__ __forceinline__ void lsm_crit_check_body(const uint32_t* __restrict__ tab, const double* __restrict__ betas,
+                                                    const double* __restrict__ cK, int N, int is_put, double K,
+                                                    double invK, unsigned long long* mism)
+{
+    const int t = 1 + (int)blockIdx.y;
+    CritIv ia, ib;
+    ia.lo[0] = tab[(size_t)t * 8]; ia.lo[1] = tab[(size_t)t * 8 + 1]; ia.len[0] = tab[(size_t)t * 8 + 2]; ia.len[1] = tab[(size_t)t * 8 + 3];
+    ib.lo[0] = tab[(size_t)t * 8 + 4]; ib.lo[1] = tab[(size_t)t * 8 + 5]; ib.len[0] = tab[(size_t)t * 8 + 6]; ib.len[1] = tab[(size_t)t * 8 + 7];
+    if (ia.lo[0] == kCritIrregular || ib.lo[0] == kCritIrregular) return;
+    double b0, b1, b2;
+    crit_fits(betas, t, N, b0, b1, b2);
+    const CritStored pa{K, invK, b0, b1, b2, is_put};
+    const CritPartner pb{K, cK[t], b0, b1, b2, is_put};
+    unsigned ma = 0, mb = 0;
+    const uint64_t n = (uint64_t)kCritTop + 1, stride = (uint64_t)gridDim.x * blockDim.x;
+    for (uint64_t o = (uint64_t)blockIdx.x * blockDim.x + threadIdx.x; o < n; o += stride) {
+        const uint32_t bits = (uint32_t)o;
+        const float s = __uint_as_float(bits);
+        ma += pa(s) != crit_in(ia, bits);
+        mb += pb(s) != crit_in(ib, bits);
+    }
+    if (ma) atomicAdd(mism + 2 * t, (unsigned long long)ma);
+    if (mb) atomicAdd(mism + 2 * t + 1, (unsigned long long)mb);
+}
 
 template <int VEC, bool WRITE_STATE>
 __device__ __forceinline__ void lsm_pass2_body(Pass2Args a)
@@ -782,45 +920,53 @@
     if (tid < 64 && (tid & 7) == 0) a.part[(size_t)(tid >> 3) * a.pstride + blockIdx.x] = s;
 }
 
-template <int VEC, int PUT = -1>
+template <int VEC, int PUT = -1, bool TAB = false>
 __device__ __forceinline__ void lsm_pass2_fold_body(Pass2Args a)
 {
     if ((int)blockIdx.x >= a.nblk) return;
     __shared__ double red[kNQ * kRedStride];
     extern __shared__ double sh_b[];
+    uint32_t* sh_t = reinterpret_cast<uint32_t*>(sh_b);
     const int tid = threadIdx.x;
     const int N = a.N;
-    if (a.gmom) {
-        for (int t = tid; t <= N; t += kBlock) {
-            double m[8], beta[3] = {0.0, 0.0, 0.0};
-            const bool inner = t >= 1 && t < N;
-#pragma unroll
-            for (int q = 0; q < 8; ++q) m[q] = inner ? a.gmom[(size_t)t * 8 + q] : 0.0;
-            if (inner) solve_poly2(m, beta);
-            const bool fit = inner && m[0] > 0.5;
-            sh_b[4 * t] = fit ? beta[0] : __builtin_huge_val();
-            sh_b[4 * t + 1] = fit ? beta[1] : 0.0;
-            sh_b[4 * t + 2] = fit ? beta[2] : 0.0;
-            sh_b[4 * t + 3] = a.cK[t];
-            if (blockIdx.x == 0 && inner && a.betas_out) {
-                double* bo = a.betas_out + (size_t)t * 4;
-                bo[0] = beta[0]; bo[1] = beta[1]; bo[2] = beta[2]; bo[3] = m[0];
-            }
-        }
+    bool irr_any = false;
+    if (TAB) {
+        irr_any = crit_load_tables(a.crit, sh_t, N);
     } else {
-        for (int k = tid; k < (N + 1) * 4; k += kBlock) {
-            const int t = k >> 2;
-            const bool fit = t >= 1 && t < N && a.betas[(size_t)t * 4 + 3] > 0.5;
-            sh_b[k] = (k & 3) == 3 ? a.cK[t] : (fit ? a.betas[k] : ((k & 3) == 0 ? __builtin_huge_val() : 0.0));
-        }
-    }
-    __syncthreads();
+        if (a.gmom) {
+            for (int t = tid; t <= N; t += kBlock) {
+                double m[8], beta[3] = {0.0, 0.0, 0.0};
+                const bool inner = t >= 1 && t < N;
+#pragma unroll
+                for (int q = 0; q < 8; ++q) m[q] = inner ? a.gmom[(size_t)t * 8 + q] : 0.0;
+                if (inner) solve_poly2(m, beta);
+                const bool fit = inner && m[0] > 0.5;
+                sh_b[4 * t] = fit ? beta[0] : __builtin_huge_val();
+                sh_b[4 * t + 1] = fit ? beta[1] : 0.0;
+                sh_b[4 * t + 2] = fit ? beta[2] : 0.0;
+                sh_b[4 * t + 3] = a.cK[t];
+                if (blockIdx.x == 0 && inner && a.betas_out) {
+                    double* bo = a.betas_out + (size_t)t * 4;
+                    bo[0] = beta[0]; bo[1] = beta[1]; bo[2] = beta[2]; bo[3] = m[0];
+                }
+            }
+        } else {
+            for (int k = tid; k < (N + 1) * 4; k += kBlock) {
+                const int t = k >> 2;
+                const bool fit = t >= 1 && t < N && a.betas[(size_t)t * 4 + 3] > 0.5;
+                sh_b[k] = (k & 3) == 3 ? a.cK[t] : (fit ? a.betas[k] : ((k & 3) == 0 ? __builtin_huge_val() : 0.0));
+            }
+        }
+        __syncthreads();
+    }
     const double K = a.K, invK = a.invK;
     const int is_put = PUT < 0 ? a.is_put : PUT;
     double acc[8];
 #pragma unroll
     for (int q = 0; q < 8; ++q) acc[q] = 0.0;
     const int64_t stride = (int64_t)a.nblk * kBlock * VEC;
+    auto sweep = [&](auto chk) {
+    constexpr bool CHK = decltype(chk)::value;
     for (int64_t j = ((int64_t)blockIdx.x * kBlock + tid) * VEC; j < a.M; j += stride) {
         float sxa[VEC], sxb[VEC];
         int32_t texa[VEC], texb[VEC];
@@ -830,8 +976,7 @@
             sxb[v] = sxa[v];
             texa[v] = texb[v] = N;
         }
-        auto decide = [&](const float (&row)[VEC], int t) {
-            const double b0 = sh_b[4 * t], b1 = sh_b[4 * t + 1], b2 = sh_b[4 * t + 2], ck = sh_b[4 * t + 3];
+        auto decide_f64 = [&](const float (&row)[VEC], int t, double b0, double b1, double b2, double ck) {
 #pragma unroll
             for (int v = 0; v < VEC; ++v) {
                 const double sd = (double)row[v];
@@ -849,13 +994,41 @@
                 texb[v] = exb ? t : texb[v];
             }
         };
+        auto decide = [&](const float (&row)[VEC], int t) {
+            if constexpr (!TAB) {
+                decide_f64(row, t, sh_b[4 * t], sh_b[4 * t + 1], sh_b[4 * t + 2], sh_b[4 * t + 3]);
+            } else {
+                const uint4 ta = *reinterpret_cast<const uint4*>(sh_t + 8 * t);
+                if (CHK && __builtin_amdgcn_readfirstlane(ta.x) == kCritIrregular) {
+                    double b0, b1, b2;
+                    crit_fits(a.betas, t, N, b0, b1, b2);
+                    decide_f64(row, t, b0, b1, b2, a.cK[t]);
+                    return;
+                }
+                const uint4 tb = *reinterpret_cast<const uint4*>(sh_t + 8 * t + 4);
+#pragma unroll
+                for (int v = 0; v < VEC; ++v) {
+                    const uint32_t bits = __float_as_uint(row[v]);
+                    const bool ex = (texa[v] == N) & (((bits - ta.x) < ta.z) | ((bits - ta.y) < ta.w));
+                    sxa[v] = ex ? row[v] : sxa[v];
+                    texa[v] = ex ? t : texa[v];
+                    const bool exb = (texb[v] == N) & (((bits - tb.x) < tb.z) | ((bits - tb.y) < tb.w));
+                    sxb[v] = exb ? row[v] : sxb[v];
+                    texb[v] = exb ? t : texb[v];
+                }
+            }
+        };
         auto live = [&]() {
             bool l = false;
 #pragma unroll
             for (int v = 0; v < VEC; ++v) l |= (texa[v] == N) | (texb[v] == N);
             return l;
         };
+#ifdef OMC_P2_U
+        constexpr int U = OMC_P2_U;
+#else
         constexpr int U = 8;
+#endif
         int t = N - 1;
         const float* col = a.S + j;
         auto fetch = [&](float (&b)[U][VEC], int tt) {
@@ -864,8 +1037,10 @@
         };
         auto work = [&](const float (&b)[U][VEC], int tt) {
 #pragma unroll
-            for (int k = 0; k < U; ++k)
+            for (int k = 0; k < U; ++k) {
                 if (tt - k >= 1) decide(b[k], tt - k);
+                if (TAB) __builtin_amdgcn_sched_barrier(0);
+            }
         };
         float bA[U][VEC], bB[U][VEC];
         if (t >= 1) fetch(bA, t);
@@ -885,7 +1060,7 @@
             double p = payoff_d(sxa[v], K, is_put);
             p = p > 0.0 ? p : 0.0;
             const double cf = p * a.D[texa[v] - 1];
-            double pb = fold_pay(fold_u(sh_b[4 * texb[v] + 3], sxb[v]), K, is_put);
+            double pb = fold_pay(fold_u(TAB ? a.cK[texb[v]] : sh_b[4 * texb[v] + 3], sxb[v]), K, is_put);
             pb = pb > 0.0 ? pb : 0.0;
             const double cfb = pb * a.D[texb[v] - 1];
             acc[0] += cf;
@@ -898,6 +1073,9 @@
             acc[3] += (cfb == 0.0) ? 1.0 : 0.0;
         }
     }
+    };
+    if (TAB && irr_any) sweep(std::true_type{});
+    else sweep(std::false_type{});
     const double s = block_reduce8(acc, red);
     if (tid < 64 && (tid & 7) == 0) a.part[(size_t)(tid >> 3) * a.pstride + blockIdx.x] = s;
 }
```

Result: faster. 666.9 billion, median of 6 (+4.3%).
